# danielzgtg/TTS.cpp

Hardware: AMD Instinct MI355X
Metric: audio-sec/wall-sec (RTF^-1), Parler-TTS-mini v1 Q4_K AR decode + DAC decode (higher is better)
Workload: dtype q4_K weights x q8_K activations (int dot, f32 combine); DAC f16 im2col x f32 weights, f64 accumulate

## Files before the change

### include/tts_hip.h

```cpp
#ifndef TTS_HIP_H
#define TTS_HIP_H

#include <stddef.h>
#include <stdint.h>

#ifdef __cplusplus
extern "C" {
#endif

#define TTS_MAX_DIMS 4
#define TTS_MAX_SRC 4
#define TTS_MAX_OP_PARAMS 16
#define TTS_MAX_NAME 64

enum tts_type {
    TTS_TYPE_F32 = 0,
    TTS_TYPE_F16 = 1,
    TTS_TYPE_Q4_0 = 2,
    TTS_TYPE_Q4_1 = 3,
    TTS_TYPE_Q5_0 = 6,
    TTS_TYPE_Q5_1 = 7,
    TTS_TYPE_Q8_0 = 8,
    TTS_TYPE_Q8_1 = 9,
    TTS_TYPE_Q4_K = 12,
// ... 122 lines not shown
const char * tts_hip_backend_name(tts_hip_backend_t backend);

void * tts_hip_buffer_alloc(tts_hip_backend_t backend, size_t size);
void tts_hip_buffer_free(tts_hip_backend_t backend, void * ptr);
size_t tts_hip_buffer_alignment(void);

int tts_hip_tensor_set(tts_hip_backend_t backend, void * dst_dev, const void * src_host, size_t size);
int tts_hip_tensor_get(tts_hip_backend_t backend, void * dst_host, const void * src_dev, size_t size);
int tts_hip_tensor_copy(tts_hip_backend_t backend, void * dst_dev, const void * src_dev, size_t size);
int tts_hip_copy_stream(tts_hip_backend_t backend, void * dst_dev, const void * src_dev, size_t size);
int tts_hip_plan_stats(tts_tensor * const * nodes, int n_nodes, int mask, int32_t * counts);
int tts_hip_tensor_set_async(tts_hip_backend_t backend, void * dst_dev, const void * src_host, size_t size);
int tts_hip_memset(tts_hip_backend_t backend, void * dst_dev, int value, size_t size);
int tts_hip_synchronize(tts_hip_backend_t backend);

int tts_hip_weight_set(tts_hip_backend_t backend, tts_tensor * t, const void * src_host);
int tts_hip_weight_get(tts_hip_backend_t backend, const tts_tensor * t, void * dst_host);
int tts_hip_quantize(tts_hip_backend_t backend, int type, const float * x_dev, void * dst_dev, int64_t rows, int64_t K);
void tts_repack_q4_K(const void * src, void * dst, int64_t nblocks, int inverse);
void tts_repack_q4_K_tiled(const void * src, void * dst, int64_t nrows, int64_t nb, int inverse);

int tts_hip_supports_op(const tts_tensor * node);
int tts_hip_graph_compute(tts_hip_backend_t backend, tts_tensor * const * nodes, int n_nodes);
int tts_hip_graph_prepare(tts_hip_backend_t backend, tts_tensor * const * nodes, int n_nodes, int slot);
int tts_hip_graph_launch(tts_hip_backend_t backend, int slot);

enum tts_hip_option {
    TTS_HIP_OPT_FUSION = 0,
    TTS_HIP_OPT_PROFILE_GEMV = 1,
    TTS_HIP_OPT_GRAPHS = 2,
    TTS_HIP_OPT_CONV_F32ACC = 3,
    TTS_HIP_OPT_CONVT_LDS = 4,
    TTS_HIP_OPT_ATTN_SPLIT = 5,
    TTS_HIP_OPT_KV_PREFETCH = 6,
    TTS_HIP_OPT_KV_PREFETCH_BLOCKS = 7,
    TTS_HIP_OPT_Q4K_TILE_BYTES = 8,
    TTS_HIP_OPT_GEMV_DEBUG = 10,
    TTS_HIP_OPT_CONV_SPLIT = 12,
    TTS_HIP_OPT_GEMV_UNIQUE = 11,
    TTS_HIP_OPT_GEMV_KS = 13,
    TTS_HIP_OPT_ATTN_FUSED = 14,
    TTS_HIP_OPT_GEMM_Q8 = 18,
    TTS_HIP_OPT_BGEMM_F32 = 19,
    TTS_HIP_OPT_CU_PARTITION = 20,
    TTS_HIP_OPT_Q4K_DUAL_BYTES = 16,
    TTS_HIP_OPT_GEMV_RSPLIT = 17,
    TTS_HIP_OPT_ATTN_PV16 = 15,
    TTS_HIP_OPT_GEMV_PREQUANT = 21,
    TTS_HIP_OPT_GEMV_KRELAY = 22,
    TTS_HIP_OPT_ATTN_KS = 23,
    TTS_HIP_OPT_ATTN_PV8 = 24,
    TTS_HIP_OPT_GEMV_KRELAY_LOOP = 26,
    TTS_HIP_OPT_GEMV_Q80_PRO = 27,
    TTS_HIP_OPT_GEMV_Q80_SLAB = 28,
    TTS_HIP_OPT_GEMV_Q80_RW = 29,
    TTS_HIP_OPT_GEMM_Q8_STAGED = 30,
    TTS_HIP_OPT_GEMV_KR_INKERNEL = 31,
    TTS_HIP_OPT_GEMV_F32_WIDE = 32,
    TTS_HIP_OPT_ATTN_PV_MP = 33,
    TTS_HIP_OPT_GEMM_KR_INKERNEL = 35,
    TTS_HIP_OPT_GEMM_KR_CT2 = 36,
    TTS_HIP_OPT_GEMM_KR_NW = 34,
    TTS_HIP_OPT_GEMV_NW_MIN = 25,
    TTS_HIP_OPT_GEMM_KR_XCD = 38,
    TTS_HIP_OPT_GEMM_KR_CP = 39,
    TTS_HIP_OPT_GEMM_KR_WALK = 40,
    TTS_HIP_OPT_GEMM_PF = 41,
    TTS_HIP_OPT_GEMM_PF_NW = 42,
    TTS_HIP_OPT_ATTN_ONE = 43,
    TTS_HIP_OPT_GEMV_KR_TAIL = 44,
    TTS_HIP_OPT_GEMV_Q50_SLAB = 45,
    TTS_HIP_OPT_GEMV_Q50_RW = 46,
    TTS_HIP_OPT_GEMM_Q5 = 47,
    TTS_HIP_OPT_GEMM_Q5_STAGED = 48,
    TTS_HIP_OPT_GEMV_Q40_SLAB = 49,
    TTS_HIP_OPT_GEMV_Q40_RW = 50,
    TTS_HIP_OPT_GEMM_Q4_0 = 51,
    TTS_HIP_OPT_GEMM_Q4_0_STAGED = 52,
    TTS_HIP_OPT_CONV_VFMA = 53,
    TTS_HIP_OPT_CONV_TILE96 = 54,
    TTS_HIP_OPT_CONV_PACK = 55,
    TTS_HIP_OPT_CONVT_PACK = 56,
    TTS_HIP_OPT_CONV_XREG = 57,
    TTS_HIP_OPT_COALESCE = 37,
};
enum tts_fuse_bits {
    TTS_FUSE_LN = 1, TTS_FUSE_GROUP = 2, TTS_FUSE_KV = 4, TTS_FUSE_EPI = 8, TTS_FUSE_HEADS = 16, TTS_FUSE_ATTN = 32,
    TTS_FUSE_LSTM = 64,
    TTS_FUSE_SNAKE = 128,
    TTS_FUSE_EMBED = 256,
    TTS_FUSE_CONV = 512,
    TTS_FUSE_ADAIN = 1024,
    TTS_FUSE_XATTN = 2048,
    TTS_FUSE_MCPY = 4096,
    TTS_FUSE_CONTREAD = 8192
};
int tts_hip_set_option(tts_hip_backend_t backend, int option, int value);
int tts_hip_attn_decode(tts_hip_backend_t backend, const tts_tensor * q, const tts_tensor * k, const tts_tensor * v,
                        const float * mask, int64_t mbs, float scale, float * out, float * out2, const int64_t * koff,
                        const int64_t * voff, const int64_t * moff, const int32_t * pseq);
int tts_hip_coalesce_stats(int device, int64_t * out, int n);
void tts_hip_coalesce_set_wait(int us);
int tts_hip_coalesce_enable(int on);
#define TTS_HIP_HOOK_FAULT_WEIGHT_SET 1
int tts_hip_test_hook(int hook, int value);
int tts_hip_install_crash_handler(void);
int tts_hip_gemv_stats(tts_hip_backend_t backend, int type, double * ms, int64_t * launches, double * bytes, int reset);
int tts_hip_greedy_step(tts_hip_backend_t backend, const float * logits, int32_t B, int32_t NH, int32_t V, int32_t step,
                        int32_t bos, int32_t eos, int32_t * eos_seen, int32_t * hist, int32_t * next);
typedef struct tts_sampling {
    float temperature;
    float top_p;
    float repetition_penalty;
    int32_t top_k;
    int32_t do_sample;
    int32_t pad_;
    uint64_t seed;
} tts_sampling;
void tts_sampling_default(tts_sampling * cfg);
uint32_t tts_sampler_call_seed(uint64_t seed, int32_t stream, int64_t call);
int tts_sampler_sample(const tts_sampling * cfg, const float * logits, int32_t NH, int32_t V, uint32_t call_seed, int32_t * last,
                       int32_t * count, int32_t * out);
int tts_hip_sample_step(tts_hip_backend_t backend, const float * logits, int32_t B, int32_t NH, int32_t V, const tts_sampling * cfg,
                        int64_t call, int32_t * rep_state, int32_t step, int32_t bos, int32_t eos, int32_t * eos_seen, int32_t * hist,
                        int32_t * next);
int tts_sampling_device_ok(const tts_sampling * cfg, int32_t V);
int tts_hip_counters(tts_hip_backend_t backend, int64_t * out, int n);

int tts_hip_gemv(tts_hip_backend_t backend, int type, const void * w, const float * x, float * y,
                 int64_t K, int64_t N, int64_t M);
int tts_hip_gemv_ex(tts_hip_backend_t backend, int type, const void * w, const float * x, float * y,
                    int64_t K, int64_t N, int64_t M, int32_t wflags);
int tts_hip_gemv_res(tts_hip_backend_t backend, int type, const void * w, const float * x, float * y, const float * res,
                     int64_t K, int64_t N, int64_t M, int32_t wflags);

typedef struct tts_backend_iface {
    void * ctx;
    const char * name;
    void * (*alloc)(void * ctx, size_t size);
    void (*free)(void * ctx, void * ptr);
    int (*set)(void * ctx, void * dst, const void * src, size_t size);
    int (*set_tensor)(void * ctx, tts_tensor * t, const void * src);
    int (*get)(void * ctx, void * dst, const void * src, size_t size);
    int (*memset)(void * ctx, void * dst, int value, size_t size);
    int (*compute)(void * ctx, tts_tensor * const * nodes, int n_nodes);
    int (*synchronize)(void * ctx);
    int (*prepare)(void * ctx, tts_tensor * const * nodes, int n_nodes, int slot);
    int (*launch)(void * ctx, int slot);
    int (*set_async)(void * ctx, void * dst, const void * src, size_t size);
    int (*copy)(void * ctx, void * dst, const void * src, size_t size);
    int (*greedy_step)(void * ctx, const float * logits, int B, int NH, int V, int step, int bos, int eos, int32_t * eos_seen,
                       int32_t * hist, int32_t * next);
    int (*sample_step)(void * ctx, const float * logits, int B, int NH, int V, const tts_sampling * cfg, int64_t call, int32_t * rep_state,
                       int step, int bos, int eos, int32_t * eos_seen, int32_t * hist, int32_t * next);
} tts_backend_iface;

int tts_hip_backend_iface(tts_hip_backend_t backend, tts_backend_iface * out);

#ifdef __cplusplus
}
#endif

#endif
```

### tts.cpp_amd/csrc/backend.hip

```cpp
#include <cmath>
#include <atomic>
#include <cstring>
#include <map>
#include <mutex>
#include <thread>

#include "hip_internal.h"
#include <hip/hip_ext.h>

#include <dlfcn.h>
#include <execinfo.h>
#include <fcntl.h>
#include <signal.h>
#include <unistd.h>

using namespace tts;


static void build_gelu_table(uint16_t * t) {
    const float GELU_COEF_A = 0.044715f;
    const float SQRT_2_OVER_PI = 0.79788456080286535587989211986876f;
    for (int i = 0; i < 65536; ++i) {
        const float x = fp16_to_fp32_host((uint16_t)i);
        const float g = 0.5f * x * (1.0f + tanhf(SQRT_2_OVER_PI * x * (1.0f + GELU_COEF_A * x * x)));
// ... 79 lines not shown
}
void conv_pack_freed(const tts_hip_backend * be, const void * p, size_t n) {
    if (g_packs_n.load(std::memory_order_acquire) == 0) return;
    const char * a = (const char *)p;
    std::vector<float *> dead;
    {
        std::lock_guard<std::mutex> lk(g_reg_mu);
        for (auto it = g_packs.begin(); it != g_packs.end();) {
            const char * w = (const char *)it->first.w;
            if (be ? it->first.be == be : (w >= a && w < a + n)) {
                dead.push_back(it->second.img);
                g_packs_bytes.fetch_sub(it->first.floats() * sizeof(float), std::memory_order_relaxed);
                it = g_packs.erase(it);
            } else {
                ++it;
            }
        }
        if (g_packs.empty()) g_packs_lo.store(UINTPTR_MAX), g_packs_hi.store(0);
        g_packs_n.store(g_packs.size(), std::memory_order_release);
    }
    if (dead.empty()) return;
    hipDeviceSynchronize();
    for (float * c : dead) hipFree(c);
}
bool buffer_lookup(const void * p, const char ** base, size_t * size) {
    std::lock_guard<std::mutex> lk(g_reg_mu);
    auto it = g_buffers.upper_bound((const char *)p);
    if (it == g_buffers.begin()) return false;
    --it;
    if ((const char *)p >= it->first + it->second.size) return false;
    if (base) *base = it->first;
    if (size) *size = it->second.size;
    return true;
}
}

extern "C" {

int tts_hip_coalesce_enable(int on) { return tts::g_coalesce_on.exchange(on ? 1 : 0); }

int tts_hip_device_count(void) {
    int n = 0;
    if (hipGetDeviceCount(&n) != hipSuccess) return 0;
    return n;
}

tts_hip_backend_t tts_hip_backend_init(int device) {
    int n = tts_hip_device_count();
    if (device < 0 || device >= n) return nullptr;
    if (hipSetDevice(device) != hipSuccess) return nullptr;
    auto * be = new tts_hip_backend();
    be->device = device;
    TTS_HIP_CHECK(hipStreamCreateWithFlags(&be->stream, hipStreamNonBlocking));
    TTS_HIP_CHECK(hipStreamCreateWithFlags(&be->cap_stream, hipStreamNonBlocking));
    TTS_HIP_CHECK(hipStreamCreateWithFlags(&be->pf_stream, hipStreamNonBlocking));
    TTS_HIP_CHECK(hipEventCreateWithFlags(&be->co_ev, hipEventDisableTiming));
    TTS_HIP_CHECK(hipEventCreateWithFlags(&be->pf_fork, hipEventDisableTiming));
    TTS_HIP_CHECK(hipEventCreateWithFlags(&be->pf_join, hipEventDisableTiming));
    hipDeviceProp_t prop;
    TTS_HIP_CHECK(hipGetDeviceProperties(&prop, device));
    snprintf(be->name, sizeof(be->name), "HIP%d(%s)", device, prop.gcnArchName);
    be->cu_total = prop.multiProcessorCount > 0 ? prop.multiProcessorCount : 256;
    be->cus = be->cu_total;
    TTS_HIP_CHECK(hipMalloc((void **)&be->scratch, kScratchBytes));
    be->scratch_size = kScratchBytes;
    TTS_HIP_CHECK(hipMalloc((void **)&be->shadow, kShadowBytes));
    be->shadow_size = kShadowBytes;
    be->hoist_size = (size_t)8 << 20;
    TTS_HIP_CHECK(hipMalloc(&be->hoist, be->hoist_size));
    TTS_HIP_CHECK(hipMalloc((void **)&be->lstm_buf, kLstmFloats * sizeof(float)));
    TTS_HIP_CHECK(hipMalloc((void **)&be->attn_buf, kAttnFloats * sizeof(float)));
    be->attn_floats = kAttnFloats;
    TTS_HIP_CHECK(hipMalloc((void **)&be->vec_scratch, kVecScratchFloats * sizeof(float)));
    be->conv_stage_floats = (size_t)8 << 20;
    TTS_HIP_CHECK(hipMalloc((void **)&be->conv_stage, be->conv_stage_floats * sizeof(float)));
    if (const char * e = getenv("TTS_HIP_OPT_CONV_VFMA"))
        if (e[0] >= '0' && e[0] <= '2' && !e[1]) be->conv_vfma = e[0] - '0';
    if (const char * e = getenv("TTS_HIP_OPT_CONV_PACK"))
        if (e[0] >= '0' && e[0] <= '1' && !e[1]) be->conv_pack = e[0] - '0';
    if (const char * e = getenv("TTS_HIP_OPT_CONVT_PACK"))
        if (e[0] >= '0' && e[0] <= '1' && !e[1]) be->convt_pack = e[0] - '0';
    if (const char * e = getenv("TTS_HIP_OPT_CONV_XREG"))
        if (e[0] >= '0' && e[0] <= '1' && !e[1]) be->conv_xreg = e[0] - '0';
    be->conv_part_doubles = (size_t)8 << 20;
    TTS_HIP_CHECK(hipMalloc((void **)&be->conv_part, be->conv_part_doubles * sizeof(double)));
    be->lstm_floats = kLstmFloats;
    TTS_HIP_CHECK(hipMalloc((void **)&be->argmax_keys, kArgmaxRows * sizeof(unsigned long long)));
    TTS_HIP_CHECK(hipMalloc((void **)&be->argmax_counts, kArgmaxRows * sizeof(unsigned)));
    TTS_HIP_CHECK(hipMemset(be->argmax_keys, 0, kArgmaxRows * sizeof(unsigned long long)));
    TTS_HIP_CHECK(hipMemset(be->argmax_counts, 0, kArgmaxRows * sizeof(unsigned)));
    TTS_HIP_CHECK(hipHostMalloc((void **)&be->pin, kPinBytes, hipHostMallocDefault));
    be->pin_size = kPinBytes;
    for (auto & e : be->plan_ev) TTS_HIP_CHECK(hipEventCreateWithFlags(&e, hipEventDisableTiming));
    std::vector<uint16_t> tab(65536);
    build_gelu_table(tab.data());
    TTS_HIP_CHECK(hipMalloc((void **)&be->gelu_table, 65536 * sizeof(uint16_t)));
    TTS_HIP_CHECK(hipMemcpy(be->gelu_table, tab.data(), 65536 * sizeof(uint16_t), hipMemcpyHostToDevice));
    return be;
}

void tts_hip_backend_free(tts_hip_backend_t be) {
    if (!be) return;
    tts::coalesce_backend_gone(be);
    hipSetDevice(be->device);
    hipStreamSynchronize(be->stream);
    tts::conv_pack_freed(be, nullptr, 0);
    for (auto & p : be->ev_pending) {
        hipEventDestroy(p.first);
        hipEventDestroy(p.second);
    }
    for (auto e : be->ev_free) hipEventDestroy(e);
    for (auto & r : be->pin_pending) hipEventDestroy(r.ev);
    for (auto e : be->pin_events) hipEventDestroy(e);
    for (auto e : be->plan_ev) hipEventDestroy(e);
    hipHostFree(be->pin);
    if (be->rb_host) hipHostFree(be->rb_host);
    hipFree(be->scratch);
    hipFree(be->shadow);
    hipFree(be->argmax_keys);
    hipFree(be->argmax_counts);
    hipFree(be->lstm_buf);
    hipFree(be->hoist);
    hipFree(be->attn_buf);
    hipFree(be->vec_scratch);
    hipFree(be->conv_stage);
    hipFree(be->conv_part);
    hipFree(be->gelu_table);
    if (be->sample_cand) hipFree(be->sample_cand);
    if (be->repack_tmp) hipFree(be->repack_tmp);
    for (char * r : be->repack_retired) hipFree(r);
    if (be->attn_stage) hipFree(be->attn_stage);
    for (auto & ex : be->gsig_exec)
        if (ex) hipGraphExecDestroy(ex);
    for (auto & ex : be->pexec)
        if (ex) hipGraphExecDestroy(ex);
    hipStreamDestroy(be->stream);
    hipStreamDestroy(be->cap_stream);
    hipStreamDestroy(be->pf_stream);
    hipEventDestroy(be->pf_fork);
    hipEventDestroy(be->pf_join);
    hipEventDestroy(be->co_ev);
    delete be;
}

const char * tts_hip_backend_name(tts_hip_backend_t be) { return be ? be->name : "HIP(null)"; }

int tts_hip_device_memory(int device, size_t * free_bytes, size_t * total_bytes) {
    if (device < 0 || device >= tts_hip_device_count()) return TTS_STATUS_NO_DEVICE;
    int prev = 0;
    hipGetDevice(&prev);
    hipSetDevice(device);
    size_t f = 0, t = 0;
    const hipError_t e = hipMemGetInfo(&f, &t);
    hipSetDevice(prev);
    if (e != hipSuccess) return TTS_STATUS_FAILED;
    if (free_bytes) *free_bytes = f;
    if (total_bytes) *total_bytes = t;
    return 0;
}

void * tts_hip_event_new(int device) {
    if (device < 0 || device >= tts_hip_device_count()) return nullptr;
    hipSetDevice(device);
    hipEvent_t ev = nullptr;
    if (hipEventCreateWithFlags(&ev, hipEventDisableTiming) != hipSuccess) return nullptr;
    return (void *)ev;
// ... 618 lines not shown
        case TTS_HIP_OPT_GEMM_Q8_STAGED:
            if (value < 0 || value > 2) return TTS_STATUS_BAD_ARG;
            be->gemm_q8_staged = value;
            return 0;
        case TTS_HIP_OPT_GEMV_Q80_RW:
            if (value < 0 || value > 32 || (value & (value - 1))) return TTS_STATUS_BAD_ARG;
            be->gemv_q80_rw = value;
            return 0;
        case TTS_HIP_OPT_GEMV_Q50_SLAB: be->gemv_q50_slab = value != 0; return 0;
        case TTS_HIP_OPT_GEMV_Q50_RW:
            if (value < 0 || value > 32 || (value & (value - 1))) return TTS_STATUS_BAD_ARG;
            be->gemv_q50_rw = value;
            return 0;
        case TTS_HIP_OPT_GEMM_Q5: be->gemm_q5 = value != 0; return 0;
        case TTS_HIP_OPT_GEMM_Q5_STAGED:
            if (value < 0 || value > 2) return TTS_STATUS_BAD_ARG;
            be->gemm_q5_staged = value;
            return 0;
        case TTS_HIP_OPT_GEMV_Q40_SLAB: be->gemv_q40_slab = value != 0; return 0;
        case TTS_HIP_OPT_GEMV_Q40_RW:
            if (value < 0 || value > 32 || (value & (value - 1))) return TTS_STATUS_BAD_ARG;
            be->gemv_q40_rw = value;
            return 0;
        case TTS_HIP_OPT_GEMM_Q4_0: be->gemm_q4_0 = value != 0; return 0;
        case TTS_HIP_OPT_GEMM_Q4_0_STAGED:
            if (value < 0 || value > 2) return TTS_STATUS_BAD_ARG;
            be->gemm_q4_0_staged = value;
            return 0;
        case TTS_HIP_OPT_ATTN_KS: be->attn_ks = value; return 0;
        case TTS_HIP_OPT_GEMV_NW_MIN: be->gemv_nw_min = value; return 0;
        case TTS_HIP_OPT_ATTN_PV8: be->attn_pv8 = value != 0; return 0;
        case TTS_HIP_OPT_GEMM_KR_CT2: be->gemm_kr_ct2 = value != 0; return 0;
        case TTS_HIP_OPT_GEMM_KR_INKERNEL: be->gemm_kr_ink = value < 0 ? 0 : value; return 0;
        case TTS_HIP_OPT_ATTN_PV_MP: be->attn_pv_mp = value == 2 ? 2 : value != 0; return 0;
        case TTS_HIP_OPT_ATTN_ONE:
            if (value < 0 || value > 2) return TTS_STATUS_BAD_ARG;
            be->attn_one = value;
            return 0;
        case TTS_HIP_OPT_GEMV_KR_TAIL:
            if (value < 0 || value > 4) return TTS_STATUS_BAD_ARG;
            be->gemv_kr_tail = value;
            return 0;
        case TTS_HIP_OPT_GEMM_KR_NW: be->gemm_kr_nw = value == 8 ? 8 : 4; return 0;
        case TTS_HIP_OPT_GEMM_Q8: be->gemm_q8 = value != 0; return 0;
        case TTS_HIP_OPT_CU_PARTITION: {
            const int count = value & 0xFF, index = (value >> 8) & 0xFF;
            const bool inter = (value >> 16) & 1;
            hipSetDevice(be->device);
            TTS_HIP_CHECK(hipStreamSynchronize(be->stream));
            hipStream_t ns = nullptr;
            if (count <= 1) {
                TTS_HIP_CHECK(hipStreamCreateWithFlags(&ns, hipStreamNonBlocking));
                be->cus = be->cu_total;
            } else {
                if (index >= count) return TTS_STATUS_BAD_ARG;
                std::vector<uint32_t> mask((be->cu_total + 31) / 32, 0u);
                const int per = be->cu_total / count;
                int n = 0;
                for (int c = 0; c < be->cu_total; ++c) {
                    const bool on = inter ? (c % count == index) : (c / per == index && c < per * count);
                    if (on) mask[c / 32] |= 1u << (c % 32), ++n;
                }
                if (hipExtStreamCreateWithCUMask(&ns, (uint32_t)mask.size(), mask.data()) != hipSuccess) return TTS_STATUS_FAILED;
                be->cus = n;
            }
            TTS_HIP_CHECK(hipStreamDestroy(be->stream));
            be->stream = ns;
            for (auto & ex : be->gsig_exec)
                if (ex) hipGraphExecDestroy(ex), ex = nullptr;
            for (auto & g : be->gsig) g = 0;
            return 0;
        }
        case TTS_HIP_OPT_BGEMM_F32: be->bgemm_f32 = value != 0; return 0;
        case TTS_HIP_OPT_GEMV_F32_WIDE: be->gemv_f32_wide = value != 0; return 0;
        case TTS_HIP_OPT_GEMV_DEBUG: be->gemv_dbg = value; return 0;
        case TTS_HIP_OPT_GEMV_UNIQUE: be->gemv_unique = value != 0; return 0;
        case TTS_HIP_OPT_GEMV_KS: be->gemv_ks_tiles = value > 0 ? value : 0; return 0;
        case TTS_HIP_OPT_COALESCE: be->co_member = value != 0; return 0;
        case TTS_HIP_OPT_GEMM_KR_XCD: be->gemm_kr_xcd = value != 0; return 0;
        case TTS_HIP_OPT_GEMM_KR_CP: be->gemm_kr_cp = value != 0; return 0;
        case TTS_HIP_OPT_GEMM_KR_WALK: be->gemm_kr_walk = value < 0 ? 0 : value; return 0;
        case TTS_HIP_OPT_GEMM_PF: be->gemm_pf = value < 0 ? 0 : value; return 0;
        case TTS_HIP_OPT_GEMM_PF_NW: be->gemm_pf_nw = value == 8 ? 8 : 4; return 0;
        case TTS_HIP_OPT_KV_PREFETCH_BLOCKS: be->kv_prefetch_blocks = value > 0 ? value : 1; return 0;
        default: return TTS_STATUS_BAD_ARG;
    }
}

extern "C" int tts_hip_counters(tts_hip_backend_t be, int64_t * out, int n) {
    if (!be || !out) return TTS_STATUS_BAD_ARG;
    const int64_t v[10] = {be->graph_updates, be->graph_instantiations, be->lstm_chains, be->lstm_steps, be->plan_wait_ns,
                           be->cap_plan_ns, be->cap_launch_ns, be->cap_update_ns, (int64_t)g_packs_n.load(), (int64_t)g_packs_bytes.load()};
    int k = 0;
    for (; k < n && k < 10; ++k) out[k] = v[k];
    return k;
}

extern "C" int tts_hip_gemv_stats(tts_hip_backend_t be, int type, double * ms, int64_t * launches, double * bytes, int reset) {
    if (!be) return TTS_STATUS_BAD_ARG;
    hipSetDevice(be->device);
    TTS_HIP_CHECK(hipStreamSynchronize(be->stream));
    for (size_t i = 0; i < be->ev_pending.size(); ++i) {
        float t = 0;
        TTS_HIP_CHECK(hipEventElapsedTime(&t, be->ev_pending[i].first, be->ev_pending[i].second));
        const int ty = be->ev_type[i];
        be->gemv_ms[ty] += t;
        be->gemv_launches[ty] += 1;
        be->gemv_bytes[ty] += be->ev_bytes[i];
        be->ev_free.push_back(be->ev_pending[i].first);
        be->ev_free.push_back(be->ev_pending[i].second);
    }
    be->ev_pending.clear();
    be->ev_bytes.clear();
    be->ev_type.clear();
    double a = 0, c = 0;
    int64_t b = 0;
    for (int ty = 0; ty < TTS_TYPE_COUNT; ++ty) {
        if (type >= 0 && ty != type) continue;
        a += be->gemv_ms[ty];
        b += be->gemv_launches[ty];
        c += be->gemv_bytes[ty];
    }
    if (ms) *ms = a;
    if (launches) *launches = b;
    if (bytes) *bytes = c;
    if (reset) {
        for (int ty = 0; ty < TTS_TYPE_COUNT; ++ty) {
            be->gemv_ms[ty] = 0;
            be->gemv_launches[ty] = 0;
            be->gemv_bytes[ty] = 0;
        }
    }
    return 0;
}

static void * hb_alloc(void * c, size_t n) { return tts_hip_buffer_alloc((tts_hip_backend_t)c, n); }
static void hb_free(void * c, void * p) { tts_hip_buffer_free((tts_hip_backend_t)c, p); }
static int hb_set(void * c, void * d, const void * s, size_t n) { return tts_hip_tensor_set((tts_hip_backend_t)c, d, s, n); }
static int hb_set_tensor(void * c, tts_tensor * t, const void * s) { return tts_hip_weight_set((tts_hip_backend_t)c, t, s); }
static int hb_get(void * c, void * d, const void * s, size_t n) { return tts_hip_tensor_get((tts_hip_backend_t)c, d, s, n); }
static int hb_memset(void * c, void * d, int v, size_t n) { return tts_hip_memset((tts_hip_backend_t)c, d, v, n); }
static int hb_compute(void * c, tts_tensor * const * nodes, int n) { return tts_hip_graph_compute((tts_hip_backend_t)c, nodes, n); }
static int hb_sync(void * c) { return tts_hip_synchronize((tts_hip_backend_t)c); }
static int hb_prepare(void * c, tts_tensor * const * nodes, int n, int slot) {
    return tts_hip_graph_prepare((tts_hip_backend_t)c, nodes, n, slot);
}
static int hb_launch(void * c, int slot) { return tts_hip_graph_launch((tts_hip_backend_t)c, slot); }
static int hb_set_async(void * c, void * d, const void * s, size_t n) { return tts_hip_tensor_set_async((tts_hip_backend_t)c, d, s, n); }
static int hb_copy(void * c, void * d, const void * s, size_t n) { return tts_hip_tensor_copy((tts_hip_backend_t)c, d, s, n); }
static int hb_greedy(void * c, const float * l, int B, int NH, int V, int step, int bos, int eos, int32_t * seen, int32_t * hist, int32_t * next) {
    return tts_hip_greedy_step((tts_hip_backend_t)c, l, B, NH, V, step, bos, eos, seen, hist, next);
}
static int hb_sample(void * c, const float * l, int B, int NH, int V, const tts_sampling * cfg, int64_t call, int32_t * rep, int step, int bos,
                     int eos, int32_t * seen, int32_t * hist, int32_t * next) {
    return tts_hip_sample_step((tts_hip_backend_t)c, l, B, NH, V, cfg, call, rep, step, bos, eos, seen, hist, next);
}

extern "C" int tts_hip_backend_iface(tts_hip_backend_t be, tts_backend_iface * out) {
    if (!be || !out) return TTS_STATUS_BAD_ARG;
    out->ctx = be;
    out->name = be->name;
    out->alloc = hb_alloc;
    out->free = hb_free;
    out->set = hb_set;
    out->set_tensor = hb_set_tensor;
    out->get = hb_get;
    out->memset = hb_memset;
    out->compute = hb_compute;
    out->synchronize = hb_sync;
    out->prepare = hb_prepare;
    out->launch = hb_launch;
    out->set_async = hb_set_async;
    out->copy = hb_copy;
    out->greedy_step = hb_greedy;
    out->sample_step = hb_sample;
    return 0;
}
// ... 1 lines not shown
```

### tts.cpp_amd/csrc/graph_exec.hip

```cpp
#include <algorithm>
#include <cstring>
#include <deque>
#include <unordered_map>
#include <vector>

#include <array>

#include "hip_internal.h"
#include <chrono>

using namespace tts;

namespace tts {
void launch_kv_prefetch(tts_hip_backend * be, hipStream_t st, const TD & t, int pdim, int blocks);
void launch_gemv_q4K_xattn(tts_hip_backend * be, const GemvJob & j, const XAttnArgs & a);
void launch_attn_decode(tts_hip_backend * be, const TD & q, const TD & k, const TD & v, const float * mask, float scale,
                        float * out, int hd, int P, int H, int n, int B, float * out2, int64_t obs = -1, int64_t mbs = 0,
                        const int64_t * koff = nullptr, const int64_t * voff = nullptr, const int64_t * moff = nullptr,
                        const int * pseq = nullptr);
void launch_attn_bias(tts_hip_backend * be, const TD & q, const TD & k, const TD & v, const float * bias, const float * mask,
                      float scale, float * out, int P, int H, int n);
void launch_layernorm(tts_hip_backend * be, const tts_tensor * dst, const tts_tensor * x, const float * w, const float * b,
                      float eps, bool rms);
}
// ... 28 lines not shown
    return t->nb[0] == es && t->nb[1] == t->nb[0] * (size_t)(t->ne[0] / tts_blck_size(t->type)) &&
           t->nb[2] == t->nb[1] * (size_t)t->ne[1] && t->nb[3] == t->nb[2] * (size_t)t->ne[2];
}

bool persistent_mem(const tts_tensor * t) {
    for (int hop = 0; t && hop < 8; ++hop) {
        if (t->op == TTS_OP_NONE || (t->flags & TTS_FLAG_PERSIST)) return true;
        if (!is_view(t->op)) return false;
        t = t->view_src ? t->view_src : t->src[0];
    }
    return false;
}

bool is_1d_f32(const tts_tensor * t, int64_t n) {
    return t->type == TTS_TYPE_F32 && t->ne[0] == n && t->ne[1] == 1 && t->ne[2] == 1 && t->ne[3] == 1 && t->nb[0] == 4;
}

float opf(const tts_tensor * t, int i) {
    float f;
    memcpy(&f, &t->op_params[i], 4);
    return f;
}

static int64_t nel(const tts_tensor * t) { return t->ne[0] * t->ne[1] * t->ne[2] * t->ne[3]; }

bool is_gemv(const tts_tensor * n) {
    const tts_tensor * a = n->src[0];
    const tts_tensor * b = n->src[1];
    if (a->ne[2] != 1 || a->ne[3] != 1) return false;
    if (b->type != TTS_TYPE_F32 || b->nb[0] != 4) return false;
    if (b->ne[2] * b->ne[3] != 1 && !(b->nb[2] == b->nb[1] * (size_t)b->ne[1] && b->nb[3] == b->nb[2] * (size_t)b->ne[2]))
        return false;
    if (n->nb[0] != 4 || (n->ne[2] * n->ne[3] != 1 && !(n->nb[2] == n->nb[1] * (size_t)n->ne[1] && n->nb[3] == n->nb[2] * (size_t)n->ne[2])))
        return false;
    if (a->nb[0] != tts_type_size(a->type)) return false;
    if ((a->type == TTS_TYPE_F16 || a->type == TTS_TYPE_F32) && b->ne[1] * b->ne[2] * b->ne[3] > 64) return false;
    if (a->type == TTS_TYPE_F16 && b->ne[1] * b->ne[2] * b->ne[3] > 8 && a->ne[0] % 8 == 0 && (b->nb[1] % 16) == 0 &&
        ((uintptr_t)b->data % 16) == 0 && (a->nb[1] % 16) == 0)
        return false;
    switch (a->type) {
        case TTS_TYPE_Q4_K:
        case TTS_TYPE_Q6_K: return a->ne[0] % 256 == 0;
        case TTS_TYPE_Q8_0:
        case TTS_TYPE_Q5_0:
        case TTS_TYPE_Q4_0: return a->ne[0] % 32 == 0;
        case TTS_TYPE_F32:
        case TTS_TYPE_F16: return a->ne[0] % 4 == 0 && (b->nb[1] % 16) == 0 && ((uintptr_t)b->data % 16) == 0;
        default: return false;
    }
}

struct GemvTarget {
    float * y;
    int64_t ycs, yrs;
    int32_t rg = 0, nrep = 1;
    int64_t rgs = 0, rep = 0;
    const tts_tensor * yt = nullptr;
};

struct Item {
    enum Kind { GEMV, ATTN, LN, LSTM, SNAKE, EMBED, CONV, ADAIN, MCPY, RINT, NODE, COPY } kind;
    const void * cp_src = nullptr;
    void * cp_dst = nullptr;
    size_t cp_bytes = 0;
    tts_tensor node{};
    const tts_tensor * rope = nullptr;
    std::vector<const tts_tensor *> mms;
    std::vector<GemvTarget> tgt;
    int epi = EPI_NONE;
    const tts_tensor * res = nullptr;
    bool ln = false;
    const tts_tensor *lnx = nullptr, *lnw = nullptr, *lnb = nullptr, *lndst = nullptr;
    float lneps = 0.f;
    bool lnrms = false;
    bool x_shadow = false;
    const tts_tensor * snake_one = nullptr;
    const tts_tensor * snake_mask = nullptr;
    bool gather_t = false;
    const tts_tensor * gt_codes = nullptr;
    const tts_tensor * xsrc = nullptr;
    bool shadow = false;
    int xattn = -1;
    bool fused = false;
    const tts_tensor *q = nullptr, *k = nullptr, *v = nullptr, *mask = nullptr, *out = nullptr;
    const tts_tensor * bias = nullptr;
    bool stage = false;
    float scale = 1.f;
    const tts_tensor *x = nullptr, *w = nullptr, *b = nullptr, *dst = nullptr;
    float eps = 0.f;
    bool rms = false;
    std::vector<const tts_tensor *> terms;
    int lkind = 0;
    LstmStepArgs ls{}, ls2{};
    bool lpair = false;
    const tts_tensor *lfinal = nullptr, *lfinal2 = nullptr;
    const float *lhist = nullptr, *lhist2 = nullptr;
    int64_t lHd = 0, lT = 0;
    const void * lstash_src[4] = {};
    void * lstash_dst[4] = {};
    size_t lstash_bytes = 0;
    Conv1dArgs conv{};
    AdainArgs adain{};
    bool rint_cpy = false;
    int rint = 1;
};

struct SmallIdx {
    int inl[3];
    std::vector<int> more;
    int n = 0;
    void push_back(int v) {
        if (n < 3) inl[n] = v;
        else more.push_back(v);
        ++n;
    }
    size_t size() const { return (size_t)n; }
    int operator[](size_t i) const { return i < 3 ? inl[i] : more[i - 3]; }
    struct iter {
        const SmallIdx * s;
        size_t i;
        int operator*() const { return (*s)[i]; }
        iter & operator++() {
            ++i;
            return *this;
        }
        bool operator!=(const iter & o) const { return i != o.i; }
        bool operator==(const iter & o) const { return i == o.i; }
        using iterator_category = std::input_iterator_tag;
        using value_type = int;
        using difference_type = std::ptrdiff_t;
        using pointer = const int *;
        using reference = int;
    };
    iter begin() const { return {this, 0}; }
    iter end() const { return {this, (size_t)n}; }
};

template <typename V>
struct PtrMap {
    struct Entry {
        const tts_tensor * first;
        V second;
    };
    std::vector<Entry> entries;
    std::vector<int32_t> slots;
    size_t mask_ = 0;
    void reserve(size_t n) {
        size_t cap = 64;
        while (cap < 2 * n) cap <<= 1;
        slots.assign(cap, -1);
        mask_ = cap - 1;
        entries.clear();
        entries.reserve(n);
    }
    size_t slot(const tts_tensor * k) const {
        uint64_t h = (uint64_t)(uintptr_t)k * 0x9E3779B97F4A7C15ull;
        size_t i = (size_t)(h >> 32) & mask_;
        while (slots[i] >= 0 && entries[slots[i]].first != k) i = (i + 1) & mask_;
        return i;
    }
    V & operator[](const tts_tensor * k) {
        if (slots.empty()) reserve(64);
        size_t i = slot(k);
        if (slots[i] < 0) {
            if (2 * (entries.size() + 1) > slots.size()) {
                std::vector<Entry> old;
// ... 52 lines not shown
            if (is_view(nodes[k]->op) || std::find(own.begin(), own.end(), k) != own.end()) continue;
            if (overlap(nodes[k], t)) return true;
        }
        return false;
    }
    const tts_tensor * sole_consumer(const tts_tensor * t) {
        auto it = consumers.find(t);
        if (it == consumers.end() || it->second.size() != 1 || uses[t] != 1) return nullptr;
        if (nodes[it->second[0]] == t) return nullptr;
        return nodes[it->second[0]];
    }
    int next_real(int i) {
        for (int j = i + 1; j < n; ++j)
            if (!is_view(nodes[j]->op)) return j;
        return -1;
    }

    void build(tts_tensor * const * nodes_, int n_) {
        const auto t_build0 = std::chrono::steady_clock::now();
        nodes = nodes_;
        n = n_;
        act.assign(n, 0);
        index.reserve((size_t)n);
        consumers.reserve((size_t)n * 2);
        for (int i = 0; i < n; ++i) {
            index[nodes[i]] = i;
            for (int s = 0; s < TTS_MAX_SRC; ++s) {
                const tts_tensor * x = nodes[i]->src[s];
                if (!x) continue;
                bool dup = false;
                for (int s2 = 0; s2 < s; ++s2) dup |= nodes[i]->src[s2] == x;
                if (dup) continue;
                consumers[x].push_back(i);
            }
        }
        for (int i = 0; i < n; ++i)
            if (read_after(nodes[i]) && !is_view(nodes[i]->op)) consumers[nodes[i]].push_back(i);
        static const bool timing = getenv("TTS_PLAN_TIMING") != nullptr;
        auto t_last = t_build0;
        char tbuf[512];
        int tlen = 0;
        auto tmark = [&](const char * what) {
            if (!timing) return;
            const auto now = std::chrono::steady_clock::now();
            tlen += snprintf(tbuf + tlen, sizeof(tbuf) - (size_t)tlen, " %s %.3f", what, std::chrono::duration<double, std::milli>(now - t_last).count());
            t_last = now;
        };
        tmark("index");
        if (mask & TTS_FUSE_LSTM) try_lstm();
        tmark("lstm");
        if (mask & TTS_FUSE_MCPY)
            for (int i = n - 1; i >= 0; --i)
                if (act[i] == 0 && nodes[i]->op == TTS_OP_CONCAT) try_rint(i);
        tmark("rint");
        if (mask & TTS_FUSE_EMBED)
            for (int i = n - 1; i >= 0; --i)
                if (act[i] == 0 && nodes[i]->op == TTS_OP_ADD) try_embed(i);
        tmark("embed");
        for (int i = 0; i < n; ++i) {
            if (act[i] != 0) continue;
            const tts_tensor * t = nodes[i];
            switch (t->op) {
                case TTS_OP_NORM:
                    if ((mask & TTS_FUSE_ADAIN) && try_adain(i)) break;
                    if (mask & TTS_FUSE_LN) try_ln(i);
                    break;
                case TTS_OP_RMS_NORM: if (mask & TTS_FUSE_LN) try_ln(i); break;
                case TTS_OP_SOFT_MAX: if (mask & TTS_FUSE_ATTN) try_attn(i); break;
                case TTS_OP_ADD: if (mask & TTS_FUSE_SNAKE) try_snake(i); break;
                case TTS_OP_IM2COL: if (mask & TTS_FUSE_CONV) try_conv(i); break;
                case TTS_OP_CPY: if (mask & TTS_FUSE_MCPY) try_mcpy(i); break;
                case TTS_OP_CONT: if (mask & TTS_FUSE_EMBED) try_gather_t(i); break;
                case TTS_OP_MUL_MAT:
                    if (!((mask & TTS_FUSE_HEADS) && try_heads(i)) && (mask & (TTS_FUSE_GROUP | TTS_FUSE_KV | TTS_FUSE_EPI))) try_gemv(i);
                    break;
                default: break;
            }
        }
        tmark("patterns");
        if (mask & TTS_FUSE_CONTREAD) skip_cont_reads();
        if (mask & TTS_FUSE_LN) fuse_ln_into_gemv();
        link_attn_shadow();
        if (mask & TTS_FUSE_XATTN) fuse_xattn();
        tmark("post");
        if (timing) fprintf(stderr, "plan %d nodes ms:%s\n", n, tbuf);
    }

    void link_attn_shadow() {
        for (int i = 0; i < n; ++i) {
            const int a = act[i];
            if (a <= 0 || items[a - 1].kind != Item::ATTN) continue;
            const int nx = next_real(i);
            if (nx < 0 || act[nx] <= 0) continue;
            Item & A = items[a - 1];
            Item & G = items[act[nx] - 1];
            if (A.bias) continue;
            if (G.kind != Item::GEMV || G.ln || G.mms[0]->src[0]->type != TTS_TYPE_Q4_K) continue;
            const tts_tensor * x = G.mms[0]->src[1];
            if (x->data != A.out->data || !contiguous(x) || tbytes(x) != tbytes(A.out)) continue;
            A.shadow = G.x_shadow = true;
        }
    }

    void fuse_xattn() {
        for (size_t ai = 0; ai < items.size(); ++ai) {
            Item & A = items[ai];
            if (A.kind != Item::ATTN || A.bias || A.k->ne[1] > 64 || A.q->ne[0] != 64 || A.q->ne[1] != 1) continue;
            const tts_tensor * Q = A.q;
            const tts_tensor * t = Q;
            int hops = 0;
            while (t && is_view(t->op) && t->src[0] && hops < 4) {
                if (uses[t->src[0]] != 1) break;
                t = t->src[0];
                ++hops;
            }
            if (!t || t->op != TTS_OP_MUL_MAT || uses[t] != 1) continue;
            const int gi = act[index[t]];
            if (gi <= 0) continue;
            Item & G = items[gi - 1];
            if (G.kind != Item::GEMV || G.mms.size() != 1 || G.mms[0] != t || G.epi != EPI_NONE || G.res || G.xattn >= 0) continue;
            const tts_tensor * W = t->src[0];
            const int64_t H = Q->ne[2], B = Q->ne[3];
            if (W->type != TTS_TYPE_Q4_K || (W->flags & TTS_FLAG_TILED) || W->ne[0] > 1024 || W->ne[1] != 64 * H ||
                t->ne[1] * t->ne[2] * t->ne[3] != B) continue;
            if (G.tgt[0].y != (float *)t->data || G.tgt[0].ycs != W->ne[1] || G.tgt[0].yrs != 1) continue;
            if (Q->data != t->data || Q->nb[0] != 4 || Q->nb[2] != 256 || (int64_t)Q->nb[3] != 4 * W->ne[1]) continue;
            if (A.k->ne[2] != H || A.v->ne[2] != H || B % A.k->ne[3] || B % A.v->ne[3]) continue;
            if (A.mask && A.mask->ne[0] != A.k->ne[1]) continue;
            const int g_node = index[t], o_node = index[A.out];
            bool clear = g_node < o_node;
            for (int i = g_node + 1; clear && i < o_node; ++i)
                if (act[i] > 0 || (act[i] == 0 && !is_view(nodes[i]->op))) clear = false;
            if (!clear) continue;
            G.xattn = (int)ai;
            A.fused = true;
        }
    }

    void skip_cont_reads() {
        for (int i = 0; i < n; ++i) {
            const tts_tensor * C = nodes[i];
            if (act[i] != 0 || C->op != TTS_OP_CONT || !C->src[0]) continue;
            const tts_tensor * s = C->src[0];
            if (s->type != C->type || !contiguous(s) || !contiguous(C) || uses[C] != 1) continue;
            if (s->ne[0] != C->ne[0] || s->ne[1] != C->ne[1] || s->ne[2] != C->ne[2] || s->ne[3] != C->ne[3]) continue;
            if (C->flags & (TTS_FLAG_OUTPUT | TTS_FLAG_PERSIST)) continue;
            const int r = next_real(i);
            if (r < 0 || act[r] != 0) continue;
            const tts_tensor * R = nodes[r];
            if (R->src[0] != C || (R->op != TTS_OP_ROPE && R->op != TTS_OP_UNARY)) continue;
            bool other = false;
            for (int si = 1; si < TTS_MAX_SRC; ++si) other |= R->src[si] == C;
            bool same = R->data == s->data && R->type == s->type;
            for (int d = 0; d < 4 && same; ++d) same = R->ne[d] == s->ne[d] && R->nb[d] == s->nb[d];
            if (other || (overlap(R, s) && !same)) continue;
            Item it;
            it.kind = Item::NODE;
            it.node = *R;
            it.node.src[0] = const_cast<tts_tensor *>(s);
            act[i] = -1;
            act[r] = add_item(std::move(it));
        }
    }

    void fuse_ln_into_gemv() {
        for (int i = 0; i < n; ++i) {
            const int a = act[i];
            if (a <= 0 || items[a - 1].kind != Item::LN) continue;
            const int nx = next_real(i);
            if (nx < 0 || act[nx] <= 0) continue;
            Item & L = items[a - 1];
            Item & G = items[act[nx] - 1];
            if (G.kind != Item::GEMV || G.ln || G.mms[0]->src[1] != L.dst) continue;
            const int wt = G.mms[0]->src[0]->type;
            const tts_tensor * B = G.mms[0]->src[1];
            if (!wtype_q8k_act(wt) && !(wtype_q80_act(wt) && q80pro && B->ne[1] * B->ne[2] * B->ne[3] <= 8)) continue;
            const int64_t K = L.dst->ne[0];
            if (K % 256 || K > 4096) continue;
            if (((uintptr_t)L.w->data & 15) || (L.b && ((uintptr_t)L.b->data & 15)) || (L.dst->nb[1] & 15)) continue;
            G.ln = true;
            G.lnx = L.x;
            G.lnw = L.w;
            G.lnb = L.b;
// ... 1480 lines not shown
    }
    const tts_tensor * member(const BatchCtx & bc, const tts_tensor * t, int k) {
        if (k == 0 || !t) return t;
        auto * e = pos.find(t);
        if (!e) return nullptr;
        const int64_t c = e->second;
        const tts_tensor * nd = bc.mnodes[k][c >> 5];
        const int slot = (int)(c & 31);
        const tts_tensor * r = slot == 31 ? nd : slot == 30 ? nd->view_src : nd->src[slot];
        return r && r->op == t->op && r->type == t->type ? r : nullptr;
    }
};
static const tts_tensor * co_member(const BatchCtx & bc, const tts_tensor * t, int k) {
    return ((CoMap *)bc.comap)->member(bc, t, k);
}
static const tts_tensor * mem_root(const tts_tensor * t) { return t && t->view_src ? t->view_src : t; }
static bool owned_mem(const tts_tensor * t) {
    const tts_tensor * r = mem_root(t);
    return r && (r->op == TTS_OP_NONE || (r->flags & TTS_FLAG_PERSIST) || persistent_mem(r));
}
static bool input_mem(const tts_tensor * t) {
    const tts_tensor * r = mem_root(t);
    return r && r->op == TTS_OP_NONE && (r->flags & TTS_FLAG_INPUT) != 0;
}

static void batch_td(const BatchCtx & bc, TD & t) {
    const int64_t s = bc.stride(t.data);
    t.data = bc.win(t.data);
    if (s) {
        t.ne[3] = bc.N;
        t.nb[3] = s;
    }
}
static int batch_n(const tts_hip_backend * be) { return be->bat ? be->bat->N : 1; }

static int run_attn_item(tts_hip_backend * be, const Item & it, const ItemTab * tab = nullptr) {
    TD q = make_td(it.q), k = make_td(it.k), v = make_td(it.v);
    float * out = (float *)it.out->data;
    const float * mask = it.mask ? (const float *)it.mask->data : nullptr;
    int B = (int)it.q->ne[3], P = (int)it.k->ne[1];
    if (it.bias) {
        if (be->bat) return TTS_STATUS_UNSUPPORTED;
        const size_t ob = tbytes(it.out);
        if (it.stage && be->attn_stage_size < ob) {
            if (be->stream == be->cap_stream) return TTS_STATUS_ALLOC_FAILED;
            if (be->attn_stage) be->repack_retired.push_back((char *)be->attn_stage);
            be->attn_stage = nullptr;
            be->attn_stage_size = 0;
            const size_t nbytes = (ob + (1u << 20) - 1) & ~(size_t)((1u << 20) - 1);
            if (hipMalloc((void **)&be->attn_stage, nbytes) != hipSuccess) {
                (void)hipGetLastError();
                return TTS_STATUS_ALLOC_FAILED;
            }
            be->attn_stage_size = nbytes;
        }
        launch_attn_bias(be, q, k, v, (const float *)it.bias->data, mask, it.scale, it.stage ? be->attn_stage : out, P, (int)it.q->ne[2],
                         (int)it.q->ne[1]);
        if (it.stage) TTS_HIP_CHECK(hipMemcpyAsync(out, be->attn_stage, ob, hipMemcpyDeviceToDevice, be->stream));
        return 0;
    }
    int64_t obs = -1, mbs = it.mask && it.mask->ne[3] > 1 ? (int64_t)(it.mask->nb[3] / 4) : 0;
    if (const BatchCtx * bc = be->bat) {
        batch_td(*bc, q);
        if (tab && tab->koff) k.ne[3] = bc->N, k.nb[3] = 0;
        else batch_td(*bc, k);
        if (tab && tab->voff) v.ne[3] = bc->N, v.nb[3] = 0;
        else batch_td(*bc, v);
        obs = bc->stride(out) / 4;
        out = bc->win(out);
        if (mask && !(tab && tab->moff)) {
            mbs = bc->stride(mask) / 4;
            mask = bc->win(mask);
        }
        B = bc->N;
        if (tab && tab->pseq) P = tab->pmax;
    }
    float * out2 = it.shadow && tbytes(it.out) * (size_t)batch_n(be) <= be->shadow_size ? be->shadow : nullptr;
    launch_attn_decode(be, q, k, v, mask, it.scale, out, (int)it.q->ne[0], P, (int)it.q->ne[2], (int)it.q->ne[1], B, out2, obs, mbs,
                       tab ? tab->koff : nullptr, tab ? tab->voff : nullptr, tab ? tab->moff : nullptr, tab ? tab->pseq : nullptr);
    return 0;
}

static int run_gemv_item(tts_hip_backend * be, const Item & it, const Item * xattn = nullptr, const ItemTab * tab = nullptr,
                         const ItemTab * xtab = nullptr) {
    const tts_tensor * mm0 = it.mms[0];
    const tts_tensor * a0 = mm0->src[0];
    tts_tensor bx;
    if (it.xsrc) {
        bx = *mm0->src[1];
        bx.data = it.xsrc->data;
    }
    const tts_tensor * b = it.xsrc ? &bx : mm0->src[1];
    GemvJob j;
    j.wtype = a0->type;
    j.K = a0->ne[0];
    j.N = a0->ne[1];
    j.M = nel(b) / b->ne[0];
    j.w_row_bytes = (int64_t)a0->nb[1];
    j.x = (const float *)b->data;
    j.xcs = (int64_t)(b->nb[1] / 4);
    const BatchCtx * bc = be->bat;
    const int64_t NB = bc ? bc->N : 1;
    j.epi = it.epi;
    j.gelu = be->gelu_table;
    if (it.res) {
        j.res = (const float *)it.res->data;
        j.rcs = (int64_t)(it.res->nb[1] / 4);
    }
    const bool q80pro = wtype_q80_act(j.wtype) && j.K % QK_K == 0 && j.M <= 8 && (it.ln || be->gemv_q80_pro);
    if (wtype_q8k_act(j.wtype) || q80pro) {
        j.pro = it.ln ? PRO_LN : PRO_QUANT;
        j.tiled = (a0->flags & TTS_FLAG_TILED) ? 1 : 0;
        if (it.ln) {
            j.x = (const float *)it.lnx->data;
            j.xcs = (int64_t)(it.lnx->nb[1] / 4);
            j.lnw = (const float *)it.lnw->data;
            j.lnb = it.lnb ? (const float *)it.lnb->data : nullptr;
            j.eps = it.lneps;
            j.rms = it.lnrms ? 1 : 0;
            j.lnout = (float *)it.lndst->data;
            j.locs = (int64_t)(it.lndst->nb[1] / 4);
        }
        auto span_y = [&](size_t k, const char *& y0, const char *& y1) {
            const tts_tensor * mm = it.mms[k];
            const int64_t Mm = mm->ne[1] * mm->ne[2] * mm->ne[3];
            y0 = (const char *)it.tgt[k].y;
            y1 = y0 + 4 * (size_t)((Mm - 1) * it.tgt[k].ycs + (mm->ne[0] - 1) * it.tgt[k].yrs + 1);
        };
        const bool xs = it.x_shadow && (size_t)(4 * j.K * j.M * NB) <= be->shadow_size;
        if (xs) {
            j.x = be->shadow;
            j.xcs = j.K;
        }
        const char * x0 = (const char *)j.x;
        const char * x1 = x0 + 4 * (size_t)((j.M - 1) * j.xcs + j.K);
        const char * l0 = (const char *)j.lnout;
        const char * l1 = l0 ? l0 + 4 * (size_t)((j.M - 1) * j.locs + j.K) : nullptr;
        bool x_hit = l0 && l0 < x1 && x0 < l1;
        for (size_t k = 0; k < it.tgt.size(); ++k) {
            const char *y0, *y1;
            span_y(k, y0, y1);
            x_hit |= y0 < x1 && x0 < y1;
            if (l0 && y0 < l1 && l0 < y1) j.lnout = nullptr;
        }
        if (bc) {
            if (!xs) {
                j.xcs = bc->stride(j.x) / 4;
                j.x = bc->win(j.x);
            }
            if (j.lnout) {
                j.locs = bc->stride(j.lnout) / 4;
                j.lnout = bc->win(j.lnout);
            }
            j.M = NB;
        }
        x_hit |= ((uintptr_t)j.x & 15) != 0 || (j.xcs & 3) != 0;
        if (x_hit) {
            if (!ensure_scratch(be, (size_t)(4 * j.K * j.M))) return TTS_STATUS_ALLOC_FAILED;
            launch_copy_cols(be, (float *)be->scratch, j.x, j.K, j.xcs, j.M);
            be->aq.src = nullptr;
            j.x = (const float *)be->scratch;
            j.xcs = j.K;
        }
    } else {
        if (it.ln) return TTS_STATUS_UNSUPPORTED;
        if (bc) {
            j.xcs = bc->stride(j.x) / 4;
            j.x = bc->win(j.x);
            j.M = NB;
        }
        int st = prepare_act(be, j.wtype, j.x, j.xcs, j.K, j.M, j.aq);
        if (st) return st;
    }
    if (bc && j.res) {
        j.rcs = bc->stride(j.res) / 4;
        j.res = bc->win(j.res);
    }
    const bool tmp = a0->type == TTS_TYPE_Q4_K && !(a0->flags & TTS_FLAG_REPACKED);
    if (xattn) {
        const Item & A = *xattn;
        TD k = make_td(A.k), v = make_td(A.v);
        const char * o0 = (const char *)A.out->data;
        const char * o1 = o0 + tbytes(A.out);
        const float * xm = bc ? (const float *)(it.ln ? it.lnx->data : b->data) : j.x;
        const int64_t xmcs = bc ? 0 : j.xcs, mm = bc ? 1 : j.M;
        const char * x0 = (const char *)xm;
        const char * x1 = x0 + 4 * (size_t)((mm - 1) * xmcs + j.K);
        const bool ok = !tmp && !j.tiled && j.wtype == TTS_TYPE_Q4_K && j.K <= 1024 && j.N == 64 * A.q->ne[2] && k.nb[0] == 4 &&
                        (k.nb[1] % 16) == 0 && (k.nb[2] % 16) == 0 && (k.nb[3] % 16) == 0 && ((uintptr_t)k.data % 16) == 0 &&
                        A.k->ne[1] >= 1 && A.k->ne[1] <= 64 && !(o0 < x1 && x0 < o1) && contiguous(A.out);
        if (ok) {
            GemvJob jj = j;
            jj.nmat = 1;
            jj.W[0] = (const uint8_t *)weight_ptr(be, a0);
            jj.Y[0] = nullptr;
            if (jj.lnout) {
                const char * l0 = it.ln ? (const char *)it.lndst->data : (const char *)jj.lnout;
                const char * l1 = l0 + 4 * (size_t)((mm - 1) * (bc ? 0 : j.locs) + j.K);
                if (l0 < o1 && o0 < l1) jj.lnout = nullptr;
            }
            XAttnArgs xa;
            xa.k = k;
            xa.v = v;
            xa.mask = A.mask ? (const float *)A.mask->data : nullptr;
            xa.scale = A.scale;
            xa.out = (float *)A.out->data;
            xa.out2 = A.shadow && tbytes(A.out) * (size_t)NB <= be->shadow_size ? be->shadow : nullptr;
            xa.P = (int)A.k->ne[1];
            xa.H = (int)A.q->ne[2];
            xa.B = (int)A.q->ne[3];
            if (bc) {
                if (xtab && xtab->koff) xa.k.ne[3] = NB, xa.k.nb[3] = 0;
                else batch_td(*bc, xa.k);
                if (xtab && xtab->voff) xa.v.ne[3] = NB, xa.v.nb[3] = 0;
                else batch_td(*bc, xa.v);
                if (xtab && xtab->moff) {
                    xa.moff = xtab->moff;
                } else {
                    xa.mbs = bc->stride(xa.mask) / 4;
                    xa.mask = bc->win(xa.mask);
                }
                xa.koff = xtab ? xtab->koff : nullptr;
                xa.voff = xtab ? xtab->voff : nullptr;
                if (xtab && xtab->pseq) xa.pseq = xtab->pseq, xa.P = xtab->pmax;
                xa.obs = bc->stride(xa.out) / 4;
                xa.out = bc->win(xa.out);
                xa.B = (int)NB;
            }
            launch_gemv_q4K_xattn(be, jj, xa);
            return 0;
        }
    }
    bool all_tl = j.wtype == TTS_TYPE_Q4_K && !tmp, any_tiled = false;
    int64_t rows = 0;
    for (const tts_tensor * mm : it.mms) {
        const int f = mm->src[0]->flags;
        all_tl &= (f & (TTS_FLAG_TILED | TTS_FLAG_TILED_COPY)) != 0;
        any_tiled |= (f & TTS_FLAG_TILED) != 0;
        rows += mm->src[0]->ne[1];
    }
    const bool use_copy = all_tl && (any_tiled || (j.M >= 8 && rows >= 2048 && j.K >= 2048));
    if (use_copy) j.tiled = 1;
    size_t k = 0;
    while (k < it.mms.size()) {
        GemvJob jj = j;
        jj.nmat = 0;
        jj.hetero = 0;
        jj.roff[0] = 0;
        if (bc && tab && tab->yoff) {
            jj.yoff = tab->yoff + k * NB;
            jj.yoff_ld = (int32_t)NB;
            jj.yoff_mats = (int32_t)((uint32_t)tab->yoff_mats >> k);
        }
        while (k < it.mms.size() && jj.nmat < GEMV_MAX_MATS) {
            const tts_tensor * a = it.mms[k]->src[0];
            if (jj.nmat > 0 && a->ne[1] != jj.N && !jj.tiled) break;
            if (it.tgt[k].rg > 0 && jj.rep_mat >= 0) break;
            if (jj.nmat > 0 && a->ne[1] != jj.N) jj.hetero = 1;
            jj.W[jj.nmat] = (const uint8_t *)weight_ptr(be, a, use_copy && !(a->flags & TTS_FLAG_TILED));
            jj.Y[jj.nmat] = bc ? bc->win(it.tgt[k].y) : it.tgt[k].y;
            jj.ycs[jj.nmat] = bc ? bc->stride(it.tgt[k].y) / 4 : it.tgt[k].ycs;
            jj.yrs[jj.nmat] = it.tgt[k].yrs;
            if (it.tgt[k].rg > 0) {
                jj.rep_mat = jj.nmat;
                jj.yrg = it.tgt[k].rg;
                jj.yrgs = it.tgt[k].rgs;
                jj.nrep = it.tgt[k].nrep;
                jj.yrep = it.tgt[k].rep;
            }
            if (jj.nmat == 0) jj.N = a->ne[1];
            jj.roff[jj.nmat + 1] = jj.roff[jj.nmat] + a->ne[1];
            jj.nmat++;
            k++;
            if (tmp) break;
        }
        if (jj.hetero) jj.N = 0;
        if (jj.wtype == TTS_TYPE_Q6_K && !gemv_q6k_ok(jj)) return TTS_STATUS_UNSUPPORTED;
        launch_gemv_job(be, jj);
    }
    if (xattn) return run_attn_item(be, *xattn, xtab);
    return 0;
}

__global__ void k_gather_t(float * __restrict__ dst, const char * __restrict__ w, int64_t wnb1, const char * __restrict__ ids,
                           int64_t inb1, int64_t T, int64_t C) {
    for (int64_t e = (int64_t)blockIdx.x * blockDim.x + threadIdx.x; e < T * C; e += (int64_t)gridDim.x * blockDim.x) {
        const int64_t c = e / T, t = e - c * T;
        const int32_t id = *(const int32_t *)(ids + t * inb1);
        dst[e] = *(const float *)(w + (int64_t)id * wnb1 + 4 * c);
    }
}

static void launch_gather_t(tts_hip_backend * be, const tts_tensor * dst, const tts_tensor * w, const tts_tensor * ids) {
    const int64_t T = dst->ne[0], C = dst->ne[1];
    int64_t g = (T * C + 255) / 256;
    if (g > 4096) g = 4096;
    hipLaunchKernelGGL(k_gather_t, dim3((unsigned)g), dim3(256), 0, be->stream, (float *)dst->data, (const char *)w->data,
                       (int64_t)w->nb[1], (const char *)ids->data, (int64_t)ids->nb[1], T, C);
    TTS_HIP_CHECK(hipGetLastError());
}

static int run_node(tts_hip_backend * be, const tts_tensor * n);

static bool batch_tensor(const BatchCtx & bc, const tts_tensor * t, tts_tensor & o) {
    o = *t;
    const int64_t s = bc.stride(t->data);
    o.data = bc.win(t->data);
    if (!s) return true;
    if (t->ne[3] != 1) return false;
    o.ne[3] = bc.N;
    o.nb[3] = (size_t)s;
    return true;
}

static int run_node_coalesced(tts_hip_backend * be, const tts_tensor * n) {
    const BatchCtx & bc = *be->bat;
    bool per_slice = false;
    switch (n->op) {
        case TTS_OP_ADD: case TTS_OP_SUB: case TTS_OP_MUL: case TTS_OP_DIV: case TTS_OP_SQR: case TTS_OP_SQRT: case TTS_OP_SIN:
        case TTS_OP_COS: case TTS_OP_SCALE: case TTS_OP_CLAMP: case TTS_OP_LEAKY_RELU: case TTS_OP_UNARY: case TTS_OP_ROUND:
        case TTS_OP_MOD: case TTS_OP_NORM: case TTS_OP_RMS_NORM: case TTS_OP_CONT: case TTS_OP_CPY: case TTS_OP_DUP:
            per_slice = true;
            break;
        case TTS_OP_CONCAT: per_slice = n->op_params[0] < 3; break;
        default: break;
    }
    tts_tensor t, srcs[TTS_MAX_SRC];
    if (per_slice && !owned_mem(n) && bc.stride(n->data) && batch_tensor(bc, n, t)) {
        for (int i = 0; i < TTS_MAX_SRC && per_slice; ++i) {
            const tts_tensor * x = n->src[i];
            if (!x) continue;
            if (input_mem(x) || (!owned_mem(x) && !bc.stride(x->data))) {
                per_slice = false;
                break;
            }
            per_slice = batch_tensor(bc, x, srcs[i]);
            if ((n->op == TTS_OP_CONT || n->op == TTS_OP_CPY || n->op == TTS_OP_DUP) && !bc.stride(x->data)) per_slice = false;
            t.src[i] = &srcs[i];
        }
        if (per_slice) return launch_op(be, &t);
    }
    BatchCtx * keep = be->bat;
    be->bat = nullptr;
    int st = 0;
    auto addr = [&](const tts_tensor * x, int k) -> void * {
        if (!owned_mem(x)) return bc.reloc(x->data, k);
        const tts_tensor * m = co_member(bc, x, k);
        return m ? m->data : nullptr;
    };
    for (int k = 0; k < bc.N && st == 0; ++k) {
        t = *n;
        t.data = addr(n, k);
        for (int i = 0; i < TTS_MAX_SRC; ++i) {
            if (!n->src[i]) continue;
            srcs[i] = *n->src[i];
            srcs[i].data = addr(n->src[i], k);
            if (!srcs[i].data) st = TTS_STATUS_FAILED;
            t.src[i] = &srcs[i];
        }
        if (!t.data) st = TTS_STATUS_FAILED;
        if (st == 0) st = run_node(be, &t);
    }
    be->bat = keep;
    return st;
}

static int run_node(tts_hip_backend * be, const tts_tensor * n) {
    if (be->bat) return run_node_coalesced(be, n);
    if (n->op == TTS_OP_MUL_MAT) {
        const tts_tensor * a = n->src[0], * b = n->src[1];
        if (a->ne[0] != b->ne[0] || b->ne[2] % a->ne[2] || b->ne[3] % a->ne[3]) return TTS_STATUS_UNSUPPORTED;
        if (is_gemv(n)) {
            Item it;
            it.kind = Item::GEMV;
            it.mms.push_back(n);
            it.tgt.push_back(GemvTarget{(float *)n->data, (int64_t)(n->nb[1] / 4), 1});
            it.tgt.back().yt = n;
            return run_gemv_item(be, it);
        }
        const int t = n->src[0]->type;
        if (t == TTS_TYPE_F32 || t == TTS_TYPE_F16) return launch_op(be, n);
        return TTS_STATUS_UNSUPPORTED;
    }
    return launch_op(be, n);
}

static int run_item(tts_hip_backend * be, const Item & it, const std::vector<Item> & items) {
    const ItemTab * tab = be->bat ? &be->bat->tabs[&it - items.data()] : nullptr;
    switch (it.kind) {
        case Item::GEMV:
            return run_gemv_item(be, it, it.xattn >= 0 ? &items[it.xattn] : nullptr, tab,
                                 be->bat && it.xattn >= 0 ? &be->bat->tabs[it.xattn] : nullptr);
        case Item::ATTN:
            if (it.fused) return 0;
            return run_attn_item(be, it, tab);
        case Item::LN:
            if (be->bat) {
                tts_tensor d, x;
                if (!batch_tensor(*be->bat, it.dst, d) || !batch_tensor(*be->bat, it.x, x)) return TTS_STATUS_UNSUPPORTED;
                launch_layernorm(be, &d, &x, (const float *)it.w->data, it.b ? (const float *)it.b->data : nullptr, it.eps, it.rms);
                return 0;
            }
            launch_layernorm(be, it.dst, it.x, (const float *)it.w->data, it.b ? (const float *)it.b->data : nullptr, it.eps, it.rms);
            return 0;
        case Item::EMBED:
            if (it.gather_t) launch_gather_t(be, it.dst, it.w, it.gt_codes);
            else launch_embed_sum(be, it.dst, it.terms.data(), (int)it.terms.size(), be->bat, tab);
            return 0;
        case Item::SNAKE:
            launch_snake(be, it.dst, it.x, it.w, it.b, it.snake_one, it.snake_mask);
            return 0;
        case Item::CONV:
            launch_conv1d_fused(be, it.conv);
            return 0;
        case Item::ADAIN:
            launch_adain_snake(be, it.adain);
            return 0;
        case Item::MCPY:
            if (it.rope) launch_rope_multi(be, it.rope, it.x, it.terms.data(), (int)it.terms.size());
            else launch_cpy_multi(be, it.x, it.terms.data(), (int)it.terms.size());
            return 0;
        case Item::RINT:
            launch_repeat_interleave1(be, it.rint_cpy ? &it.node : it.dst, it.x, it.rint);
            return 0;
        case Item::NODE:
            return run_node(be, &it.node);
        case Item::COPY:
            launch_copy_bytes(be, it.cp_dst, it.cp_src, it.cp_bytes);
            return 0;
        case Item::LSTM:
            if (it.lkind & 4)
                for (int g = 0; g < 4; ++g)
                    launch_copy_bytes(be, it.lstash_dst[g], it.lstash_src[g], it.lstash_bytes);
            if (it.lkind & 1) {
                launch_lstm_step(be, it.ls, it.lpair ? &it.ls2 : nullptr);
                be->lstm_steps += it.lpair ? 2 : 1;
            }
            if (it.lkind & 2) {
                launch_lstm_finish(be, it.lfinal, it.lhist, it.lHd, it.lT);
                be->lstm_chains++;
                if (it.lfinal2) {
                    launch_lstm_finish(be, it.lfinal2, it.lhist2, it.lHd, it.lT);
                    be->lstm_chains++;
                }
            }
            return 0;
    }
    return TTS_STATUS_FAILED;
}

bool tts::co_debug() {
    static const bool on = [] {
        const char * e = getenv("TTS_HIP_COALESCE_DEBUG");
        return e && e[0] == '1';
    }();
    return on;
}
#define CO_NO()                                                                                   \
    do {                                                                                          \
        if (tts::co_debug()) fprintf(stderr, "coalesce: step refused at graph_exec.hip:%d\n", __LINE__); \
        return false;                                                                             \
    } while (0)

static bool co_per_slice(const BatchCtx & bc, const tts_tensor * n) {
    switch (n->op) {
        case TTS_OP_ADD: case TTS_OP_SUB: case TTS_OP_MUL: case TTS_OP_DIV: case TTS_OP_SQR: case TTS_OP_SQRT: case TTS_OP_SIN:
        case TTS_OP_COS: case TTS_OP_SCALE: case TTS_OP_CLAMP: case TTS_OP_LEAKY_RELU: case TTS_OP_UNARY: case TTS_OP_ROUND:
        case TTS_OP_MOD: case TTS_OP_NORM: case TTS_OP_RMS_NORM: case TTS_OP_CONT: case TTS_OP_CPY: case TTS_OP_DUP: break;
        case TTS_OP_CONCAT:
            if (n->op_params[0] < 3) break;
            return false;
        default: return false;
    }
    if (owned_mem(n) || !bc.stride(n->data) || n->ne[3] != 1) return false;
    for (int i = 0; i < TTS_MAX_SRC; ++i) {
// ... 661 lines not shown
```

### tts.cpp_amd/csrc/hip_internal.h

```cpp
#pragma once

#include <hip/hip_fp16.h>
#include <hip/hip_runtime.h>

#include <cstdio>
#include <cstdlib>
#include <atomic>
#include <deque>
#include <mutex>
#include <unordered_map>
#include <tuple>
#include <vector>

#include "common.h"

#define TTS_HIP_CHECK(expr)                                                                          \
    do {                                                                                             \
        hipError_t err_ = (expr);                                                                    \
        if (err_ != hipSuccess) {                                                                    \
            fprintf(stderr, "%s:%d: HIP error %s: %s\n", __FILE__, __LINE__, #expr, hipGetErrorString(err_)); \
            abort();                                                                                 \
        }                                                                                            \
    } while (0)

// ... 178 lines not shown
}
#endif

struct ActQuant {
    const void * src = nullptr;
    int64_t K = 0, M = 0;
    int vtype = -1;
    int64_t graph_epoch = -1;
    int8_t * qs = nullptr;
    float * d = nullptr;
    int32_t * bsums = nullptr;
};

enum { EPI_NONE = 0, EPI_GELU = 1, EPI_ADD = 2, EPI_SWIGLU = 3, EPI_SILU_MUL = 4 };
constexpr int GEMV_MAX_MATS = 16;
struct GemvJob {
    int wtype = 0;
    int nmat = 1;
    const uint8_t * W[GEMV_MAX_MATS] = {};
    float * Y[GEMV_MAX_MATS] = {};
    int64_t w_row_bytes = 0, K = 0, N = 0, M = 0;
    int64_t ycs[GEMV_MAX_MATS] = {}, yrs[GEMV_MAX_MATS] = {};
    const float * res = nullptr;
    int64_t rcs = 0;
    int epi = EPI_NONE;
    const uint16_t * gelu = nullptr;
    const float * x = nullptr;
    int64_t xcs = 0;
    ActQuant aq;
    int pro = 0;
    int tiled = 0;
    int hetero = 0;
    int64_t roff[GEMV_MAX_MATS + 1] = {};
    int32_t rep_mat = -1, yrg = 0, nrep = 0;
    int64_t yrgs = 0, yrep = 0;
    int dbg = 0;
    const float * lnw = nullptr;
    const float * lnb = nullptr;
    float eps = 0.f;
    int rms = 0;
    float * lnout = nullptr;
    int64_t locs = 0;
    const char * bq = nullptr;
    int64_t bq_bytes = 0;
    int64_t bq_tile = 0;
    int32_t bq_slot = 0;
    unsigned long long * ts = nullptr;
    const int64_t * yoff = nullptr;
    int32_t yoff_mats = 0, yoff_ld = 0;
    int32_t xcd_cols = 0;
    int32_t kr_tail = 0;
};
enum { KR_TAIL_RES = 1, KR_TAIL_FOLD = 2, KR_TAIL_BESIDE = 4 };
constexpr int KR_FOLD_BYTES = 4 * 4 * (2 * 64 * 16 + 64 * 4);
__host__ __device__ inline int64_t job_roff(const GemvJob & j, int m) { return j.hetero ? j.roff[m] : (int64_t)m * j.N; }
__host__ __device__ inline int64_t job_rows(const GemvJob & j) { return job_roff(j, j.nmat); }
#ifdef TTS_PHASE_TS
#define TTS_TS(job, k)                                                                                            \
    do {                                                                                                          \
        if ((job).ts && (threadIdx.x & 63) == 0)                                                                  \
            (job).ts[((((size_t)blockIdx.z * gridDim.y + blockIdx.y) * gridDim.x + blockIdx.x) * (blockDim.x >> 6) + \
                      (threadIdx.x >> 6)) * 8 +                                                                   \
                     (k)] = __builtin_amdgcn_s_memrealtime();                                                     \
    } while (0)
#else
#define TTS_TS(job, k) \
    do {               \
    } while (0)
#endif
enum { PRO_QUANT = 1, PRO_LN = 2, PRO_COPY = 3 };
struct XAttnArgs {
    TD k, v;
    const float * mask = nullptr;
    float scale = 1.f;
    float * out = nullptr;
    float * out2 = nullptr;
    int P = 0, H = 0, B = 0;
    int64_t obs = 0;
    int64_t mbs = 0;
    const int64_t * koff = nullptr;
    const int64_t * voff = nullptr;
    const int64_t * moff = nullptr;
    const int * pseq = nullptr;
};

constexpr int EMBED_MAX_TERMS = 16;
struct BatchCls {
    const char * b0 = nullptr;
    size_t size = 0;
    char * win = nullptr;
    int64_t stride = 0;
};
struct ItemTab {
    const int64_t * yoff = nullptr;
    int32_t yoff_mats = 0;
    const int64_t *koff = nullptr, *voff = nullptr;
    const int64_t * moff = nullptr;
    const int * pseq = nullptr;
    int pmax = 0;
    const int64_t * ioff[EMBED_MAX_TERMS] = {};
};
struct BatchCtx {
    int N = 0;
    uint64_t key = 0;
    std::vector<BatchCls> cls;
    std::vector<tts_tensor * const *> mnodes;
    std::vector<tts_hip_backend *> mbe;
    int n_nodes = 0;
    bool checked = false;
    int canon = 0;
    bool ragged = false;
    bool differs = false;
    std::vector<ItemTab> tabs;
    void * comap = nullptr;
    const BatchCls * find(const void * p) const {
        const char * c = (const char *)p;
        size_t lo = 0, hi = cls.size();
        while (lo < hi) {
            const size_t m = (lo + hi) / 2;
            if (cls[m].b0 <= c) lo = m + 1;
            else hi = m;
        }
        if (lo == 0) return nullptr;
        const BatchCls & b = cls[lo - 1];
        return c < b.b0 + b.size ? &b : nullptr;
    }
    template <typename T>
    T * win(T * p) const {
        const BatchCls * b = p ? find(p) : nullptr;
        return b ? (T *)(b->win + ((const char *)p - b->b0)) : p;
    }
    int64_t stride(const void * p) const {
        const BatchCls * b = p ? find(p) : nullptr;
        return b ? b->stride : 0;
    }
    template <typename T>
    T * reloc(T * p, int k) const {
        const BatchCls * b = p ? find(p) : nullptr;
        return b ? (T *)(b->win + k * b->stride + ((const char *)p - b->b0)) : p;
    }
};

}

struct tts_hip_backend {
    int device = 0;
    hipStream_t stream = nullptr;
    char name[64] = {0};
    char * scratch = nullptr;
    size_t scratch_size = 0;
    float * shadow = nullptr;
    size_t shadow_size = 0;
    void * hoist = nullptr;
    size_t hoist_size = 0;
    float * attn_buf = nullptr;
    size_t attn_floats = 0;
    int attn_split_minp = 128;
    int attn_ks = 2;
    int attn_pv_mp = 1;
    int attn_one = 1;
    int attn_pv8 = 0;
    int attn_pv_uv16 = 0;
    int attn_fused_minp = 0;
    unsigned long long * argmax_keys = nullptr;
    unsigned * argmax_counts = nullptr;
    int64_t q4k_tile_bytes = 4 << 20;
    int gemv_dbg = 0;
    int gemv_unique = 1;
    int gemm_q8 = 1;
    int64_t cus = 256;
    int cu_total = 256;
    int bgemm_f32 = 1;
    int gemv_f32_wide = 1;
    int gemm_kr_nw = 4;
    int64_t gemv_ks_tiles = 256;
    int gemv_mf_prequant = 1;
    int gemv_kr = 1;
    int gemv_kr_loop = 1;
    int gemv_kr_tail = 1;
    int gemv_q80_pro = 1;
    int gemv_q80_slab = 1;
    int gemv_q80_rw = 0;
    int gemm_q8_staged = 2;
    int gemv_q50_slab = 1;
    int gemv_q50_rw = 0;
    int gemm_q5 = 1;
    int gemm_q5_staged = 2;
    int gemv_q40_slab = 1;
    int gemv_q40_rw = 0;
    int gemm_q4_0 = 1;
    int gemm_q4_0_staged = 2;
    int64_t gemv_kr_ink = 0;
    int gemm_kr_walk = 0;
    int gemm_pf = 64;
    int gemm_pf_nw = 4;
    int gemm_kr_cp = 0;
    int gemm_kr_xcd = 0;
    int gemm_kr_ct2 = 0;
    int64_t gemm_kr_ink = 0;
    int gemv_nw_min = 0;
    int gemv_mf_rsplit = 1;
    int64_t q4k_dual_bytes = 1 << 20;
    void * sample_cand = nullptr;
    size_t sample_cand_size = 0;
    int kv_prefetch_minp = 0;
    int kv_prefetch_blocks = 128;
    hipStream_t pf_stream = nullptr;
    hipEvent_t pf_fork = nullptr, pf_join = nullptr;
    uint8_t * pin = nullptr;
    size_t pin_size = 0, pin_head = 0;
    struct PinRec {
        size_t off, size;
        hipEvent_t ev;
    };
    std::deque<PinRec> pin_pending;
    std::vector<hipEvent_t> pin_events;
    std::mutex pin_mu;
    hipEvent_t plan_ev[2] = {nullptr, nullptr};
    bool plan_ev_pending[2] = {false, false};
    float * lstm_buf = nullptr;
    float * conv_stage = nullptr;
    size_t conv_stage_floats = 0;
    float * vec_scratch = nullptr;
    size_t lstm_floats = 0;
    tts::ActQuant aq;
    int64_t graph_epoch = 0;
    uint16_t * gelu_table = nullptr;
    bool convt_lds = true;
    double * conv_part = nullptr;
    size_t conv_part_doubles = 0;
    int conv_vfma = 1;
    int conv_tile96 = 1;
    int conv_pack = 1;
    int convt_pack = 1;
    int conv_xreg = 1;
    bool capturing = false;
    int conv_split = 1;
    int fusion = 0x3FFF;
    bool profile_gemv = false;
    double gemv_ms[TTS_TYPE_COUNT] = {0};
    int64_t gemv_launches[TTS_TYPE_COUNT] = {0};
    double gemv_bytes[TTS_TYPE_COUNT] = {0};
    std::vector<std::pair<hipEvent_t, hipEvent_t>> ev_pending;
    std::vector<double> ev_bytes;
    std::vector<int> ev_type;
    std::vector<hipEvent_t> ev_free;
    char * repack_tmp = nullptr;
    size_t repack_tmp_size = 0;
    std::vector<char *> repack_retired;
    float * attn_stage = nullptr;
    size_t attn_stage_size = 0;
    bool use_graphs = false;
    static constexpr int N_GSIG = 4;
    uint64_t gsig[N_GSIG] = {};
    hipGraphExec_t gsig_exec[N_GSIG] = {};
    int gsig_next = 0;
    bool conv_f32acc = false;
    int conv_acc_mode = 0;
    hipStream_t cap_stream = nullptr;
    int64_t graph_updates = 0, graph_instantiations = 0;
    int64_t lstm_chains = 0, lstm_steps = 0;
    int64_t plan_wait_ns = 0;
    int64_t cap_plan_ns = 0, cap_launch_ns = 0, cap_update_ns = 0;
    hipGraphExec_t pexec[2] = {nullptr, nullptr};
    tts_tensor * const * plan_nodes[2] = {nullptr, nullptr};
    int plan_n[2] = {0, 0};
    bool plan_eager[2] = {true, true};
    bool plan_prepared[2] = {false, false};
    tts::BatchCtx * bat = nullptr;
    hipEvent_t co_ev = nullptr;
    int64_t * co_tab = nullptr;
    size_t co_tab_bytes = 0;
    int64_t co_prep_ns = 0;
    bool co_member = true;
    struct RbEnt {
        const char * dev;
        size_t bytes, off;
// ... 159 lines not shown
```

### tts.cpp_amd/csrc/k_gemv.hip

```cpp
#include "hip_internal.h"
#include <hip/hip_ext.h>

#include <atomic>
#include <type_traits>

#ifndef TTS_GEMV_EARLY16
#define TTS_GEMV_EARLY16 1
#endif

namespace tts {

__device__ __forceinline__ int dev_nearest_int(float f) {
    const float val = __fadd_rn(f, 12582912.f);
    const int i = __float_as_int(val);
    return (i & 0x007fffff) - 0x00400000;
}

__global__ __launch_bounds__(256) void k_quantize_q8_K(const float * __restrict__ x, int64_t xcs, int64_t K,
                                                       int8_t * __restrict__ qs, float * __restrict__ dout,
                                                       int32_t * __restrict__ s32) {
    const int blk = blockIdx.x;
    const int m = blockIdx.y;
    const int t = threadIdx.x;
    const int64_t nb = K / QK_K;
// ... 1588 lines not shown
    const int P = a.pseq ? a.pseq[b] : a.P;
    const int p = min(lane, P - 1);
    float4 kr[F];
    float vv[VB];
    float mk = 0.f;
    const int bk = b / (a.B / (int)a.k.ne[3]), bv = b / (a.B / (int)a.v.ne[3]);
    const char * kbase = a.k.data + (int64_t)h * a.k.nb[2] + (int64_t)bk * a.k.nb[3] + (a.koff ? a.koff[b] : 0);
    const char * vbase = a.v.data + (int64_t)h * a.v.nb[2] + (int64_t)bv * a.v.nb[3] + (a.voff ? a.voff[b] : 0);
    u32x4 hdr[4], q[4];
    if (wave < NW) {
        const int64_t row = (int64_t)h * HD + wave * 8 + s;
        const uint8_t * wr = j.W[0] + row * j.w_row_bytes;
        auto mid = [&]() {
#pragma unroll
            for (int u = 0; u < 4; ++u) {
                const int64_t bo = (int64_t)min(u, nb - 1) * 144;
                hdr[u] = TTS_WLOAD((const u32x4 *)(wr + bo));
                q[u] = TTS_WLOAD((const u32x4 *)(wr + bo + 16 + l * 16));
            }
        };
        ProOv ov;
        ov.nwaves = NW;
        ov.xcol = j.x + (int64_t)b * j.xcs;
        ov.lncol = j.lnout && h == 0 ? j.lnout + (int64_t)b * j.locs : nullptr;
        q4k_prologue<PRO, 4>(j, nb, xq_s, xd_s, xs_s, nullptr, nullptr, mid, ov);
    } else {
#pragma unroll
        for (int c = 0; c < F; ++c) kr[c] = *(const float4 *)(kbase + (int64_t)p * a.k.nb[1] + 16 * c);
#pragma unroll
        for (int u = 0; u < VB; ++u) vv[u] = *(const float *)(vbase + (int64_t)lane * a.v.nb[1] + (int64_t)min(u, P - 1) * a.v.nb[0]);
        mk = *(a.mask ? a.mask + (a.moff ? a.moff[b] : (int64_t)b * a.mbs) + p : (const float *)kbase);
    }
    __syncthreads();
    if (wave < NW) {
        float sums = 0.f, sumf = 0.f;
#pragma unroll
        for (int u = 0; u < 4; ++u) q4k_block(hdr[u], q[u], xq_s, xs_s, xd_s, min(u, nb - 1), l, u < nb, sums, sumf);
        const float tot = q4k_octet_total(sumf, sums);
        if (l == 0) s_q[wave * 8 + s] = tot;
    }
    __syncthreads();
    if (wave != NW) return;
    double acc = 0.0;
#pragma unroll
    for (int c = 0; c < F; ++c) {
        acc += (double)__fmul_rn(kr[c].x, s_q[4 * c + 0]);
        acc += (double)__fmul_rn(kr[c].y, s_q[4 * c + 1]);
        acc += (double)__fmul_rn(kr[c].z, s_q[4 * c + 2]);
        acc += (double)__fmul_rn(kr[c].w, s_q[4 * c + 3]);
    }
    float w = __fmul_rn((float)acc, a.scale);
    if (a.mask) w = __fadd_rn(w, __fmul_rn(1.0f, mk));
    if (lane >= P) w = -INFINITY;
    float mx = w;
    mx = fmaxf(mx, dpp_f32<DPP_XOR1>(mx));
    mx = fmaxf(mx, dpp_f32<DPP_XOR2>(mx));
    mx = fmaxf(mx, dpp_f32<DPP_HALF_MIRROR>(mx));
    mx = fmaxf(mx, dpp_f32<DPP_MIRROR>(mx));
    mx = fmaxf(fmaxf(__int_as_float(__builtin_amdgcn_readlane(__float_as_int(mx), 0)), __int_as_float(__builtin_amdgcn_readlane(__float_as_int(mx), 16))),
               fmaxf(__int_as_float(__builtin_amdgcn_readlane(__float_as_int(mx), 32)), __int_as_float(__builtin_amdgcn_readlane(__float_as_int(mx), 48))));
    const float e = lane < P ? cr_expf(__fsub_rn(w, mx)) : 0.f;
    double sum = 0.0;
    for (int i = 0; i < P; ++i) sum += (double)__int_as_float(__builtin_amdgcn_readlane(__float_as_int(e), i));
    const float pr = __fmul_rn(e, (float)(1.0 / sum));
    double o = 0.0;
    for (int i0 = 0; i0 < P; i0 += VB) {
        if (i0 > 0) {
#pragma unroll
            for (int u = 0; u < VB; ++u) vv[u] = *(const float *)(vbase + (int64_t)lane * a.v.nb[1] + (int64_t)min(i0 + u, P - 1) * a.v.nb[0]);
            TTS_PIN_LOADS();
        }
#pragma unroll
        for (int u = 0; u < VB; ++u) {
            if (i0 + u >= P) break;
            const float pi = __int_as_float(__builtin_amdgcn_readlane(__float_as_int(pr), i0 + u));
            o += (double)__fmul_rn(pi, vv[u]);
        }
    }
    const int64_t orow = (int64_t)h * HD + lane;
    a.out[(int64_t)b * (a.obs ? a.obs : (int64_t)a.H * HD) + orow] = (float)o;
    if (a.out2) a.out2[(int64_t)b * a.H * HD + orow] = (float)o;
}

void launch_gemv_q4K_xattn(tts_hip_backend * be, const GemvJob & j, const XAttnArgs & a) {
    const dim3 grid((unsigned)a.H, (unsigned)a.B);
    if (j.pro == PRO_LN) hipLaunchKernelGGL(k_gemv_q4K_xattn<PRO_LN>, grid, dim3(576), 0, be->stream, j, a);
    else hipLaunchKernelGGL(k_gemv_q4K_xattn<PRO_QUANT>, grid, dim3(576), 0, be->stream, j, a);
    TTS_HIP_CHECK(hipGetLastError());
}

template <int MC, int PRO = 0>
__global__ __launch_bounds__(256) void k_gemv_q8_0(GemvJob j, int RW) {
    extern __shared__ __attribute__((aligned(16))) char smem[];
    const int nb = (int)(j.K / QK8_0);
    const int mat = blockIdx.y;
    const uint8_t * __restrict__ W = j.W[mat];
    float * Y = j.Y[mat];
    const int64_t row0 = (int64_t)blockIdx.x * RW;
    const int rows = (int)((j.N - row0) < RW ? (j.N - row0) : RW);
    const int M = j.M;
    int8_t * xq_s = (int8_t *)smem;
    float * xd_s = (float *)(smem + al16((size_t)MC * j.K + (PRO ? QK_K : 0)));
    int * s_s = (int *)((char *)xd_s + al16(sizeof(float) * (MC * nb + (PRO ? QK_K / QK8_0 : 0))));
    float * f_s = (float *)((char *)s_s + al16(sizeof(int) * (size_t)RW * nb * MC));
    const int npairs = rows * nb;
    int wv0[8];
    uint16_t dw0;
    {
        const int p = min((int)threadIdx.x, npairs - 1);
        const int r = p / nb, b = p % nb;
        const uint16_t * bp = (const uint16_t *)(W + (row0 + r) * j.w_row_bytes + (int64_t)b * 34);
        dw0 = *gptr(bp);
#pragma unroll
        for (int k = 0; k < 8; ++k) wv0[k] = (int)*gptr(bp + 1 + 2 * k) | ((int)*gptr(bp + 2 + 2 * k) << 16);
    }
    TTS_PIN_LOADS();
    if constexpr (PRO != 0) {
        q4k_prologue<PRO, 16, false, NoMid, true>(j, (int)(j.K / QK_K), xq_s, xd_s, nullptr);
    } else {
        const int4 * src = (const int4 *)j.aq.qs;
        int4 * dst = (int4 *)xq_s;
        const int n16 = (int)((int64_t)M * j.K / 16);
        for (int i = threadIdx.x; i < n16; i += 256) dst[i] = src[i];
        for (int i = threadIdx.x; i < M * nb; i += 256) xd_s[i] = j.aq.d[i];
    }
    __syncthreads();
    for (int p = threadIdx.x; p < npairs; p += 256) {
        const int r = p / nb, b = p % nb;
        float dw;
        int wv[8];
        if (p == (int)threadIdx.x) {
            dw = dev_fp16_to_fp32(dw0);
#pragma unroll
            for (int k = 0; k < 8; ++k) wv[k] = wv0[k];
        } else {
            const uint16_t * bp = (const uint16_t *)(W + (row0 + r) * j.w_row_bytes + (int64_t)b * 34);
            dw = dev_fp16_to_fp32(bp[0]);
#pragma unroll
            for (int k = 0; k < 8; ++k) wv[k] = (int)bp[1 + 2 * k] | ((int)bp[2 + 2 * k] << 16);
        }
#pragma unroll
        for (int m = 0; m < MC; ++m) {
            if (m >= M) break;
            const int4 * xb = (const int4 *)(xq_s + (m * nb + b) * QK8_0);
            const int4 x0 = xb[0], x1 = xb[1];
            int s = __builtin_amdgcn_sdot4(wv[0], x0.x, 0, false);
            s = __builtin_amdgcn_sdot4(wv[1], x0.y, s, false);
            s = __builtin_amdgcn_sdot4(wv[2], x0.z, s, false);
            s = __builtin_amdgcn_sdot4(wv[3], x0.w, s, false);
            s = __builtin_amdgcn_sdot4(wv[4], x1.x, s, false);
            s = __builtin_amdgcn_sdot4(wv[5], x1.y, s, false);
            s = __builtin_amdgcn_sdot4(wv[6], x1.z, s, false);
            s = __builtin_amdgcn_sdot4(wv[7], x1.w, s, false);
            const int o = (r * MC + m) * nb + b;
            s_s[o] = s;
            f_s[o] = __fmul_rn(dw, xd_s[m * nb + b]);
        }
    }
    __syncthreads();
    for (int t = threadIdx.x; t < rows * MC; t += 256) {
        const int r = t / MC, m = t % MC;
        if (m >= M) continue;
        float a = 0.f;
        const int o = (r * MC + m) * nb;
        for (int b = 0; b < nb; ++b) a = __fadd_rn(a, __fmul_rn((float)s_s[o + b], f_s[o + b]));
        gemv_store<MC>(j, mat, row0 + r, m, a);
    }
// ... 806 lines not shown
        j.x = job.x + m0 * job.xcs;
        for (int i = 0; i < job.nmat; ++i) j.Y[i] = job.Y[i] + m0 * job.ycs[i];
        if (job.yoff) j.yoff = job.yoff + m0;
        if (job.res) j.res = job.res + m0 * job.rcs;
        if (j.pro == PRO_LN && j.K > 4 * 1024) {
            fprintf(stderr, "tts_hip: LN-fused Q4_K GEMV with K = %lld > 4096\n", (long long)j.K);
            abort();
        }
        const int64_t nb = j.K / QK_K;
        const int64_t bq = (((j.M * nb + 1) * (2 * QK_K + 32 + 4)) + 1023) & ~(int64_t)1023;
        if (j.K <= be->gemv_kr_ink && !j.dbg) {
            GemvJob ji = j;
            ji.bq = nullptr;
            ji.bq_bytes = bq;
            if (launch_q4k_kr(be, ji)) continue;
        }
        if (be->gemv_mf_prequant && !j.dbg && (size_t)(bq + 4 * j.K * j.M) <= be->scratch_size) {
            j.bq = be->scratch + be->scratch_size - bq;
            j.bq_bytes = bq;
            const dim3 qg((unsigned)((nb + 3) / 4), (unsigned)j.M);
            if (j.pro == PRO_LN) hipLaunchKernelGGL(k_quant_mf<PRO_LN>, qg, dim3(64), 0, be->stream, j);
            else hipLaunchKernelGGL(k_quant_mf<PRO_QUANT>, qg, dim3(64), 0, be->stream, j);
            TTS_HIP_CHECK(hipGetLastError());
            j.pro = PRO_COPY;
            j.lnout = nullptr;
            if (!launch_q4k_kr(be, j)) launch_q4k_mf_pro<PRO_COPY, 16>(be, j);
            continue;
        }
        if (j.pro == PRO_LN) launch_q4k_mf_pro<PRO_LN, 16>(be, j);
        else launch_q4k_mf_pro<PRO_QUANT, 16>(be, j);
    }
}

static size_t q4k_kr_lds(int64_t bq_bytes, bool sw) { return (size_t)((bq_bytes + 15) & ~15) + (sw ? 2 * 64 * 36 * 4 + 64 * 16 : 64 * 36 * 4); }
template <int BPW, bool SW, int NWT, bool LANE = false, bool LOOP = false, int PRO = PRO_COPY, int CTW = 1, bool CP = false>
static void launch_q4k_kr_t(tts_hip_backend * be, const GemvJob & job, unsigned gx, unsigned gy = 1) {
    static const int tail_bits[5] = {0, KR_TAIL_RES | KR_TAIL_FOLD, KR_TAIL_RES | KR_TAIL_FOLD | KR_TAIL_BESIDE, KR_TAIL_RES, KR_TAIL_FOLD};
    GemvJob j = job;
    j.kr_tail = tail_bits[be->gemv_kr_tail];
    if constexpr (PRO == PRO_COPY && CTW == 1 && !CP) {
        if (j.pro == PRO_LN) return launch_q4k_kr_t<BPW, SW, NWT, LANE, LOOP, PRO_LN>(be, j, gx, gy);
        if (j.pro == PRO_QUANT) return launch_q4k_kr_t<BPW, SW, NWT, LANE, LOOP, PRO_QUANT>(be, j, gx, gy);
    }
    if constexpr (SW && !LOOP && BPW <= 3 && CTW == 1) {
        if (be->gemv_kr_loop && gx > (unsigned)be->cus && gy == 1) {
            launch_q4k_kr_t<BPW, SW, NWT, LANE, true, PRO>(be, j, (unsigned)be->cus, gy);
            return;
        }
    }
    static std::atomic<uint32_t> attr_done{0};
    set_lds_attr_once(attr_done, be->device, (const void *)k_gemv_q4K_kr<BPW, SW, NWT, LANE, LOOP, PRO, CTW, CP>);
    size_t lds = q4k_kr_lds((CP ? 2 : CTW) * (j.bq_tile ? j.bq_tile : j.bq_bytes), SW || CP);
    if constexpr (!SW && !LOOP && CTW == 1 && !CP && BPW == 1 && NWT == 4) {
        if ((j.kr_tail & KR_TAIL_FOLD) && j.K == 4 * QK_K) {
            const size_t ops = lds - 64 * 36 * 4;
            lds = (j.kr_tail & KR_TAIL_BESIDE) ? ops + KR_FOLD_BYTES : std::max(ops, (size_t)KR_FOLD_BYTES);
        }
    }
    const dim3 blk(64 * NWT * ((SW || CP) ? 2 : 1));
    if (be->profile_gemv) {
        hipEvent_t e0, e1;
        profile_pair(be, e0, e1);
        hipExtLaunchKernelGGL((k_gemv_q4K_kr<BPW, SW, NWT, LANE, LOOP, PRO, CTW, CP>), dim3(gx, gy), blk, (uint32_t)lds, be->stream, e0, e1, 0u, j);
        profile_push(be, e0, e1, gemv_bytes(j), TTS_TYPE_Q4_K);
        return;
    }
    hipLaunchKernelGGL((k_gemv_q4K_kr<BPW, SW, NWT, LANE, LOOP, PRO, CTW, CP>), dim3(gx, gy), blk, lds, be->stream, j);
}

static size_t q4k_pf_lds(int64_t nb) { return (size_t)((((16 * nb + 1) * (2 * PF_SLOT + 32 + 4)) + 1023) & ~(int64_t)1023); }
template <int NB, bool LANE, int NW>
static void launch_q4k_pf_nw(tts_hip_backend * be, const GemvJob & j, unsigned gy) {
    static std::atomic<uint32_t> attr_done{0};
    set_lds_attr_once(attr_done, be->device, (const void *)k_gemm_q4K_pf<NB, LANE, NW>);
    const unsigned gx = (unsigned)((job_rows(j) / 16 + NW * PF_RS - 1) / (NW * PF_RS));
    hipLaunchKernelGGL((k_gemm_q4K_pf<NB, LANE, NW>), dim3(gx, gy), dim3(64 * NW), (uint32_t)q4k_pf_lds(NB), be->stream, j);
}
template <int NB, bool LANE>
static void launch_q4k_pf_t(tts_hip_backend * be, const GemvJob & j, unsigned gy) {
    if (be->gemm_pf_nw == 8) launch_q4k_pf_nw<NB, LANE, 8>(be, j, gy);
    else launch_q4k_pf_nw<NB, LANE, 4>(be, j, gy);
}

static bool launch_gemm_q4k_kr(tts_hip_backend * be, const GemvJob & job, size_t lo_res = SIZE_MAX) {
    if (!be->gemv_kr || !be->gemv_mf_prequant || job.wtype != TTS_TYPE_Q4_K || job.M <= 8 || job.epi == EPI_SWIGLU || job.dbg) return false;
    if (job.pro != PRO_QUANT && job.pro != PRO_LN) return false;
    if (job.pro == PRO_LN && job.K > 4 * 1024) return false;
    const int64_t nb = job.K / QK_K;
    if (nb != 4 && nb != 8 && nb != 12 && nb != 16) return false;
    for (int m = 0; m <= job.nmat; ++m)
        if (job_roff(job, m) % 16) return false;
    const int64_t ink_m = be->gemm_kr_ink & 0xFFFF;
    const bool ink = ink_m > 0 && job.M <= ink_m && job.K <= 4 * 1024 && !job.dbg &&
                     (job.pro == PRO_LN || job.xcs == job.K) && (!(be->gemm_kr_ink & 0x10000) || job.pro == PRO_QUANT);
    const bool pf = be->gemm_pf > 0 && job.M >= be->gemm_pf && !ink;
    const int64_t tile = pf ? (int64_t)q4k_pf_lds(nb) : (((16 * nb + 1) * (2 * QK_K + 32 + 4)) + 1023) & ~(int64_t)1023;
    const int64_t nct = (job.M + 15) / 16;
    if (q4k_kr_lds(tile, false) > 160 * 1024) return false;
    const char * xs0 = (const char *)job.x;
    const char * xs1 = xs0 + 4 * (size_t)((job.M - 1) * job.xcs + job.K);
    const size_t lo = lo_res != SIZE_MAX ? lo_res
                      : (xs0 >= be->scratch && xs0 < be->scratch + be->scratch_size) ? (size_t)(xs1 - be->scratch) : 0;
    const int64_t avail = lo < be->scratch_size ? (int64_t)(be->scratch_size - lo) : 0;
    if (tile * nct > avail || (lo == 0 && (size_t)(tile * nct + 4 * job.K * job.M) > be->scratch_size) || nct > 65535) {
        const int64_t per = (lo ? avail / tile : (int64_t)be->scratch_size / (tile + 16 * 4 * job.K)) * 16;
        if (per < 16 || job.rep_mat >= 0) return false;
        for (int64_t m0 = 0; m0 < job.M; m0 += per) {
            GemvJob j = job;
            j.M = job.M - m0 < per ? job.M - m0 : per;
            if (job.lnout) j.lnout = job.lnout + m0 * job.locs;
            j.x = job.x + m0 * job.xcs;
            for (int i = 0; i < job.nmat; ++i) j.Y[i] = job.Y[i] + m0 * job.ycs[i];
        if (job.yoff) j.yoff = job.yoff + m0;
            if (job.res) j.res = job.res + m0 * job.rcs;
            if (!launch_gemm_q4k_kr(be, j, lo)) return false;
        }
        return true;
    }
    GemvJob j = job;
    j.bq_tile = tile;
    j.bq_bytes = tile * nct;
    j.bq_slot = pf ? PF_SLOT : 0;
    if (ink) {
        j.bq = nullptr;
    } else {
        j.bq = be->scratch + be->scratch_size - j.bq_bytes;
        const dim3 qg((unsigned)((nb + 3) / 4), (unsigned)j.M);
        if (j.pro == PRO_LN) hipLaunchKernelGGL(k_quant_mf<PRO_LN>, qg, dim3(64), 0, be->stream, j);
        else hipLaunchKernelGGL(k_quant_mf<PRO_QUANT>, qg, dim3(64), 0, be->stream, j);
        TTS_HIP_CHECK(hipGetLastError());
        j.pro = PRO_COPY;
        j.lnout = nullptr;
    }
    const unsigned gx = (unsigned)(job_rows(j) / 16), gy = (unsigned)nct;
    j.xcd_cols = be->gemm_kr_xcd && nct > 1 ? 1 : 0;
    const bool ct2 = be->gemm_kr_ct2 && !ink && nct >= 2 && (nb == 4 || nb == 8) && q4k_kr_lds(2 * tile, false) <= 160 * 1024;
    const bool cp = be->gemm_kr_cp && !ink && nct >= 2 && (nb == 4 || nb == 8) && q4k_kr_lds(2 * tile, true) <= 160 * 1024;
    auto go = [&](auto LANE) {
        constexpr bool L = decltype(LANE)::value;
        if (pf) {
            switch (nb) {
                case 4: launch_q4k_pf_t<4, L>(be, j, gy); break;
                case 8: launch_q4k_pf_t<8, L>(be, j, gy); break;
                case 12: launch_q4k_pf_t<12, L>(be, j, gy); break;
                default: launch_q4k_pf_t<16, L>(be, j, gy); break;
            }
            return;
        }
        if (cp) {
            const unsigned gy2 = (unsigned)((nct + 1) / 2);
            if (nb == 4) launch_q4k_kr_t<1, false, 4, L, false, PRO_COPY, 1, true>(be, j, gx, gy2);
            else launch_q4k_kr_t<2, false, 4, L, false, PRO_COPY, 1, true>(be, j, gx, gy2);
            return;
        }
        if (ct2) {
            const unsigned gy2 = (unsigned)((nct + 1) / 2);
            if (nb == 4) launch_q4k_kr_t<1, false, 4, L, false, PRO_COPY, 2>(be, j, gx, gy2);
            else launch_q4k_kr_t<2, false, 4, L, false, PRO_COPY, 2>(be, j, gx, gy2);
            return;
        }
        const int walk = be->gemm_kr_walk;
        if (walk > 0 && nct > 4 && gx > (unsigned)walk && !ink) {
            switch (nb) {
                case 4: launch_q4k_kr_t<1, false, 4, L, true>(be, j, (unsigned)walk, gy); break;
                case 8: launch_q4k_kr_t<2, false, 4, L, true>(be, j, (unsigned)walk, gy); break;
                case 12: launch_q4k_kr_t<3, false, 4, L, true>(be, j, (unsigned)walk, gy); break;
                default: launch_q4k_kr_t<4, false, 4, L, true>(be, j, (unsigned)walk, gy); break;
            }
            return;
        }
        const bool nw8 = be->gemm_kr_nw == 8;
        switch (nb) {
            case 4: launch_q4k_kr_t<1, false, 4, L>(be, j, gx, gy); break;
            case 8: nw8 ? launch_q4k_kr_t<1, false, 8, L>(be, j, gx, gy) : launch_q4k_kr_t<2, false, 4, L>(be, j, gx, gy); break;
            case 12: launch_q4k_kr_t<3, false, 4, L>(be, j, gx, gy); break;
            default: nw8 ? launch_q4k_kr_t<2, false, 8, L>(be, j, gx, gy) : launch_q4k_kr_t<4, false, 4, L>(be, j, gx, gy); break;
        }
    };
    if (j.tiled) go(std::false_type{});
    else go(std::true_type{});
    TTS_HIP_CHECK(hipGetLastError());
    return true;
}
static bool launch_q4k_kr(tts_hip_backend * be, const GemvJob & j) {
    if (!be->gemv_kr || j.M > 8) return false;
    if (j.pro != PRO_COPY && !((j.pro == PRO_QUANT || j.pro == PRO_LN) && j.K <= 4 * 1024 && !j.bq_tile)) return false;
    const bool sw = j.epi == EPI_SWIGLU;
    if (!sw) {
        for (int m = 0; m <= j.nmat; ++m)
            if (job_roff(j, m) % 16) return false;
    } else if (j.N % 16) {
        return false;
    }
    if (q4k_kr_lds(j.bq_bytes, sw) > 160 * 1024) return false;
    const int64_t T = sw ? j.N / 16 : job_rows(j) / 16;
    if (T < 1 || T > 0x7fffffff) return false;
    const unsigned gx = (unsigned)T;
    switch (j.K / QK_K) {
        case 4: sw ? launch_q4k_kr_t<1, true, 4>(be, j, gx) : launch_q4k_kr_t<1, false, 4>(be, j, gx); return true;
        case 8: sw ? launch_q4k_kr_t<2, true, 4>(be, j, gx) : launch_q4k_kr_t<2, false, 4>(be, j, gx); return true;
        case 12: sw ? launch_q4k_kr_t<3, true, 4>(be, j, gx) : launch_q4k_kr_t<3, false, 4>(be, j, gx); return true;
        case 16: sw ? launch_q4k_kr_t<4, true, 4>(be, j, gx) : launch_q4k_kr_t<4, false, 4>(be, j, gx); return true;
        case 32: if (sw) return false; launch_q4k_kr_t<4, false, 8>(be, j, gx); return true;
        default: return false;
    }
}

static size_t q4k_ks_lds(int64_t M, int64_t nb) {
// ... 1075 lines not shown
            while (RW > 1 && q80_lds(MC, j.K, RW) > 64 * 1024) RW /= 2;
            const size_t lds = q80_lds(MC, j.K, RW) + (j.pro ? QK_K + 64 : 0);
            const unsigned grid = (unsigned)((j.N + RW - 1) / RW);
            if (j.pro == PRO_LN) hipLaunchKernelGGL((k_gemv_q8_0<MC, PRO_LN>), dim3(grid, nmat), dim3(256), lds, be->stream, j, RW);
            else if (j.pro == PRO_QUANT) hipLaunchKernelGGL((k_gemv_q8_0<MC, PRO_QUANT>), dim3(grid, nmat), dim3(256), lds, be->stream, j, RW);
            else hipLaunchKernelGGL(k_gemv_q8_0<MC>, dim3(grid, nmat), dim3(256), lds, be->stream, j, RW);
        } break;
        case TTS_TYPE_F16: {
            const unsigned grid = (unsigned)((j.N + 3) / 4);
            hipLaunchKernelGGL((k_gemv_float<MC, true>), dim3(grid, nmat), dim3(256), 0, be->stream, j);
        } break;
        default: {
            const unsigned grid = (unsigned)((j.N + 3) / 4);
            hipLaunchKernelGGL((k_gemv_float<MC, false>), dim3(grid, nmat), dim3(256), 0, be->stream, j);
        } break;
    }
}

__global__ void k_spin(long long ticks) {
    const long long t0 = (long long)__builtin_amdgcn_s_memrealtime();
    while ((long long)__builtin_amdgcn_s_memrealtime() - t0 < ticks) __builtin_amdgcn_s_sleep(2);
}

void launch_profile_spin(tts_hip_backend * be, double us) {
    hipLaunchKernelGGL(k_spin, dim3(1), dim3(64), 0, be->stream, (long long)(us * 100.0));
    TTS_HIP_CHECK(hipGetLastError());
}

void launch_gemv_job(tts_hip_backend * be, const GemvJob & job) {
    const bool prof = be->profile_gemv && job.wtype != TTS_TYPE_Q4_K && !(job.wtype == TTS_TYPE_Q8_0 && job.M <= 8 && q80s_ok(be, job)) &&
                      !(job.wtype == TTS_TYPE_Q5_0 && job.M <= 8 && q50s_ok(be, job)) &&
                      !(job.wtype == TTS_TYPE_Q4_0 && job.M <= 8 && q40s_ok(be, job));
    hipEvent_t e0 = nullptr, e1 = nullptr;
    if (prof) {
        profile_pair(be, e0, e1);
        TTS_HIP_CHECK(hipEventRecord(e0, be->stream));
    }
    const int64_t K = job.K;
    if (job.wtype == TTS_TYPE_F32 && job.M > 8 && gemm_f32_ok(job)) {
        launch_gemm_f32(be, job);
        if (prof) {
            TTS_HIP_CHECK(hipEventRecord(e1, be->stream));
            profile_push(be, e0, e1, gemv_bytes(job), job.wtype);
        }
        return;
    }
    if (job.wtype == TTS_TYPE_Q8_0 && job.M > 8 && job.aq.vtype == TTS_TYPE_Q8_0 && !job.hetero && be->gemm_q8) {
        launch_gemm_q8_0(be, job);
        TTS_HIP_CHECK(hipGetLastError());
        if (prof) {
            TTS_HIP_CHECK(hipEventRecord(e1, be->stream));
            profile_push(be, e0, e1, gemv_bytes(job), job.wtype);
        }
        return;
    }
    if (job.wtype == TTS_TYPE_Q5_0 && job.M > 8 && job.aq.vtype == TTS_TYPE_Q8_0 && !job.hetero && be->gemm_q5) {
        launch_gemm_q5_0(be, job);
        TTS_HIP_CHECK(hipGetLastError());
        if (prof) {
            TTS_HIP_CHECK(hipEventRecord(e1, be->stream));
            profile_push(be, e0, e1, gemv_bytes(job), job.wtype);
        }
        return;
    }
    if (job.wtype == TTS_TYPE_Q4_0 && job.M > 8 && job.aq.vtype == TTS_TYPE_Q8_0 && !job.hetero && be->gemm_q4_0) {
        launch_gemm_q4_0(be, job);
        TTS_HIP_CHECK(hipGetLastError());
        if (prof) {
            TTS_HIP_CHECK(hipEventRecord(e1, be->stream));
            profile_push(be, e0, e1, gemv_bytes(job), job.wtype);
        }
        return;
    }
    if (job.wtype == TTS_TYPE_Q6_K) {
        launch_gemv_q6k(be, job);
        TTS_HIP_CHECK(hipGetLastError());
        if (prof) {
            TTS_HIP_CHECK(hipEventRecord(e1, be->stream));
            profile_push(be, e0, e1, gemv_bytes(job), job.wtype);
        }
        return;
    }
    if (job.M > 8 && launch_gemm_q4k_kr(be, job)) return;
    if (q4k_ks_eligible(be, job)) {
        launch_q4k_ks(be, job);
        TTS_HIP_CHECK(hipGetLastError());
        return;
    }
    if (q4k_mf_eligible(be, job)) {
        launch_q4k_mf(be, job);
        TTS_HIP_CHECK(hipGetLastError());
        return;
    }
    if (job.epi == EPI_SWIGLU) {
        fprintf(stderr, "tts_hip: SwiGLU GEMV epilogue needs the matrix-core Q4_K kernel\n");
        abort();
    }
    const int64_t cmax = job.wtype == TTS_TYPE_Q4_K ? q4k_max_cols(K) : 8;
    for (int64_t m0 = 0; m0 < job.M; m0 += cmax) {
        const int64_t mc = job.M - m0 < cmax ? job.M - m0 : cmax;
        GemvJob j = job;
        j.M = mc;
        if (job.lnout) j.lnout = job.lnout + m0 * job.locs;
        if (job.aq.vtype == TTS_TYPE_Q8_K) {
            j.aq.qs = job.aq.qs + m0 * K;
            j.aq.d = job.aq.d + m0 * (K / QK_K);
            j.aq.bsums = job.aq.bsums + m0 * (K / 32);
        } else if (job.aq.vtype == TTS_TYPE_Q8_0) {
            j.aq.qs = job.aq.qs + m0 * K;
            j.aq.d = job.aq.d + m0 * (K / QK8_0);
        } else if (job.aq.vtype == TTS_TYPE_F16) {
            j.aq.qs = job.aq.qs + m0 * K * 2;
        }
        if (job.x) j.x = job.x + m0 * job.xcs;
        for (int i = 0; i < job.nmat; ++i) j.Y[i] = job.Y[i] + m0 * job.ycs[i];
        if (job.yoff) j.yoff = job.yoff + m0;
        if (job.res) j.res = job.res + m0 * job.rcs;
        switch (mc) {
            case 1: launch_gemv_mc<1>(be, j); break;
            case 2: launch_gemv_mc<2>(be, j); break;
            case 3: case 4: launch_gemv_mc<4>(be, j); break;
            default: launch_gemv_mc<8>(be, j); break;
        }
    }
    TTS_HIP_CHECK(hipGetLastError());
    if (prof) {
        TTS_HIP_CHECK(hipEventRecord(e1, be->stream));
        profile_push(be, e0, e1, gemv_bytes(job), job.wtype);
    }
}

}
```

### tts.cpp_amd/ttship/__init__.py

```python
import ctypes
import os
import pathlib

_HERE = pathlib.Path(__file__).resolve().parent
PKG_ROOT = _HERE.parent
REPO_ROOT = PKG_ROOT.parent
LIB_PATH = PKG_ROOT / "lib" / "libtts_hip.so"

F32, F16, Q4_0, Q5_0, Q8_0, Q4_K, Q6_K, Q8_K, I32 = 0, 1, 2, 6, 8, 12, 14, 15, 26
QUANT_MIX_Q4_K_M = 1
PROF_ATTN = 39

OPS = ["NONE", "DUP", "ADD", "SUB", "MUL", "DIV", "SQR", "SQRT", "SIN", "COS", "SUM_ROWS", "REPEAT",
       "CONCAT", "NORM", "RMS_NORM", "MUL_MAT", "SCALE", "CPY", "CONT", "RESHAPE", "VIEW", "PERMUTE",
       "TRANSPOSE", "GET_ROWS", "SOFT_MAX", "ROPE", "CLAMP", "CONV_TRANSPOSE_1D", "IM2COL", "UPSCALE",
       "PAD", "LEAKY_RELU", "UNARY", "CUMSUM", "MOD", "ROUND", "STFT", "ISTFT", "MAP_CUSTOM3", "MAP_CUSTOM2"]
OP = {n: i for i, n in enumerate(OPS)}
FUSE = {"LN": 1, "GROUP": 2, "KV": 4, "EPI": 8, "HEADS": 16, "ATTN": 32, "LSTM": 64, "SNAKE": 128, "EMBED": 256, "CONV": 512, "ADAIN": 1024, "XATTN": 2048, "MCPY": 4096, "CONTREAD": 8192}
FUSE_ALL = sum(FUSE.values())
UNARY = {"ABS": 0, "NEG": 1, "TANH": 2, "RELU": 3, "SIGMOID": 4, "GELU": 5, "SILU": 6, "EXP": 7}

OPT = {"FUSION": 0, "PROFILE_GEMV": 1, "GRAPHS": 2, "CONV_F32ACC": 3, "CONVT_LDS": 4, "ATTN_SPLIT": 5, "KV_PREFETCH": 6, "KV_PREFETCH_BLOCKS": 7, "Q4K_TILE_BYTES": 8, "GEMV_DEBUG": 10, "GEMV_UNIQUE": 11, "CONV_SPLIT": 12, "GEMV_KS": 13, "ATTN_FUSED": 14, "ATTN_PV16": 15, "Q4K_DUAL_BYTES": 16, "GEMV_RSPLIT": 17, "GEMM_Q8": 18, "BGEMM_F32": 19, "CU_PARTITION": 20, "GEMV_PREQUANT": 21, "GEMV_KRELAY": 22, "ATTN_KS": 23, "ATTN_PV8": 24, "GEMV_NW_MIN": 25, "GEMV_KRELAY_LOOP": 26, "GEMV_Q80_PRO": 27, "GEMV_Q80_SLAB": 28, "GEMV_Q80_RW": 29, "GEMM_Q8_STAGED": 30, "GEMV_KR_INKERNEL": 31, "GEMV_F32_WIDE": 32, "ATTN_PV_MP": 33, "GEMM_KR_NW": 34, "GEMM_KR_INKERNEL": 35, "GEMM_KR_CT2": 36, "COALESCE": 37, "GEMM_KR_XCD": 38, "GEMM_KR_CP": 39, "GEMM_KR_WALK": 40, "GEMM_PF": 41, "GEMM_PF_NW": 42, "ATTN_ONE": 43, "GEMV_KR_TAIL": 44, "GEMV_Q50_SLAB": 45, "GEMV_Q50_RW": 46, "GEMM_Q5": 47, "GEMM_Q5_STAGED": 48, "GEMV_Q40_SLAB": 49, "GEMV_Q40_RW": 50, "GEMM_Q4_0": 51, "GEMM_Q4_0_STAGED": 52, "CONV_VFMA": 53, "CONV_TILE96": 54, "CONV_PACK": 55, "CONVT_PACK": 56, "CONV_XREG": 57}
ATTN_SPLIT_DEFAULT = 128
ATTN_ONE_DEFAULT = 1
GEMV_KR_TAIL_DEFAULT = 1
ATTN_FUSED_ON = 128

TYPE_SIZE = {F32: 4, F16: 2, Q4_K: 144, Q6_K: 210, Q8_0: 34, Q5_0: 22, Q4_0: 18, I32: 4}
BLCK_SIZE = {F32: 1, F16: 1, Q4_K: 256, Q6_K: 256, Q8_0: 32, Q5_0: 32, Q4_0: 32, I32: 1}


class TtsTensor(ctypes.Structure):
    pass


TtsTensor._fields_ = [
    ("type", ctypes.c_int32),
    ("op", ctypes.c_int32),
    ("ne", ctypes.c_int64 * 4),
    ("nb", ctypes.c_uint64 * 4),
    ("op_params", ctypes.c_int32 * 16),
    ("src", ctypes.POINTER(TtsTensor) * 4),
    ("view_src", ctypes.POINTER(TtsTensor)),
    ("view_offs", ctypes.c_uint64),
    ("data", ctypes.c_void_p),
    ("flags", ctypes.c_int32),
    ("pad_", ctypes.c_int32),
    ("name", ctypes.c_char * 64),
]


class BackendIface(ctypes.Structure):
    _fields_ = [
        ("ctx", ctypes.c_void_p),
        ("name", ctypes.c_char_p),
        ("alloc", ctypes.c_void_p),
        ("free", ctypes.c_void_p),
        ("set", ctypes.c_void_p),
        ("set_tensor", ctypes.c_void_p),
        ("get", ctypes.c_void_p),
        ("memset", ctypes.c_void_p),
        ("compute", ctypes.c_void_p),
        ("synchronize", ctypes.c_void_p),
        ("prepare", ctypes.c_void_p),
        ("launch", ctypes.c_void_p),
        ("set_async", ctypes.c_void_p),
        ("copy", ctypes.c_void_p),
        ("greedy_step", ctypes.c_void_p),
        ("sample_step", ctypes.c_void_p),
    ]


class Sampling(ctypes.Structure):
    _fields_ = [
        ("temperature", ctypes.c_float),
        ("top_p", ctypes.c_float),
        ("repetition_penalty", ctypes.c_float),
        ("top_k", ctypes.c_int32),
        ("do_sample", ctypes.c_int32),
        ("pad_", ctypes.c_int32),
        ("seed", ctypes.c_uint64),
    ]


def sampling(**kw):
    c = Sampling()
    lib().tts_sampling_default(ctypes.byref(c))
    for k, v in kw.items():
        setattr(c, k, v)
    return c


def call_seed(seed, stream, call):
    return int(lib().tts_sampler_call_seed(seed, stream, call))


def host_sample(cfg, logits, call_seed_, last=None, count=None):
    import numpy as np
    lg = np.ascontiguousarray(logits, dtype=np.float32)
    NH, V = lg.shape
    out = np.zeros(NH, dtype=np.int32)
    if last is None:
        last = np.full(NH, -1, dtype=np.int32)
    if count is None:
        count = np.zeros(NH, dtype=np.int32)
# ... 450 lines not shown
            raise RuntimeError("tts_hip_backend_iface failed")
        if reference_flow:
            for f in ("prepare", "launch", "set_async", "copy", "greedy_step", "sample_step"):
                setattr(it, f, None)
        return it

    def alloc(self, nbytes):
        p = self.L.tts_hip_buffer_alloc(self.ptr, nbytes)
        if not p:
            raise MemoryError(f"tts_hip_buffer_alloc({nbytes}) failed")
        return p

    def free(self, p):
        self.L.tts_hip_buffer_free(self.ptr, p)

    def set(self, dev, host_arr):
        st = self.L.tts_hip_tensor_set(self.ptr, dev, host_arr.ctypes.data, host_arr.nbytes)
        if st != 0:
            raise RuntimeError(f"tensor_set failed {st}")

    def get(self, host_arr, dev):
        st = self.L.tts_hip_tensor_get(self.ptr, host_arr.ctypes.data, dev, host_arr.nbytes)
        if st != 0:
            raise RuntimeError(f"tensor_get failed {st}")

    def sample_step(self, logits, cfg, call, rep_state=None, step=100, bos=-2, eos=-3, eos_seen=None):
        import numpy as np
        lg = np.ascontiguousarray(logits, dtype=np.float32)
        B, NH, V = lg.shape
        rs = np.ascontiguousarray(rep_state if rep_state is not None else np.tile(np.array([-1, 0], np.int32), B * NH), dtype=np.int32)
        es = np.ascontiguousarray(eos_seen if eos_seen is not None else np.zeros(B * NH, np.int32), dtype=np.int32)
        bufs = [self.alloc(n) for n in (lg.nbytes, rs.nbytes, es.nbytes, B * NH * 4, B * NH * 4)]
        try:
            self.set(bufs[0], lg)
            self.set(bufs[1], rs)
            self.set(bufs[2], es)
            st = self.L.tts_hip_sample_step(self.ptr, bufs[0], B, NH, V, ctypes.byref(cfg), call, bufs[1], step, bos, eos, bufs[2], bufs[3], bufs[4])
            if st != 0:
                raise RuntimeError(f"tts_hip_sample_step failed {st}")
            hist = np.zeros((B, NH), np.int32)
            nxt = np.zeros((NH, B), np.int32)
            self.get(hist, bufs[3])
            self.get(nxt, bufs[4])
            self.get(rs, bufs[1])
            self.get(es, bufs[2])
            return hist, nxt, es, rs
        finally:
            for b in bufs:
                self.free(b)

    def quantize(self, wtype, x):
        import numpy as np
        x = np.ascontiguousarray(x, dtype=np.float32)
        N, K = x.shape
        rs = K // BLCK_SIZE[wtype] * TYPE_SIZE[wtype]
        dx, dq = self.alloc(x.nbytes), self.alloc(N * rs)
        try:
            self.set(dx, x)
            st = self.L.tts_hip_quantize(self.ptr, wtype, dx, dq, N, K)
            if st != 0:
                raise RuntimeError(f"tts_hip_quantize failed {st}")
            out = np.empty(N * rs, dtype=np.uint8)
            self.get(out, dq)
            return out
        finally:
            self.free(dx)
            self.free(dq)

    def sync(self):
        if self.L.tts_hip_synchronize(self.ptr) != 0:
            raise RuntimeError("synchronize failed")

    def set_option(self, opt, value):
        self.L.tts_hip_set_option(self.ptr, opt, value)

    def gemv_stats(self, wtype=-1, reset=True):
        ms = ctypes.c_double()
        n = ctypes.c_int64()
        b = ctypes.c_double()
        self.L.tts_hip_gemv_stats(self.ptr, wtype, ctypes.byref(ms), ctypes.byref(n), ctypes.byref(b), 1 if reset else 0)
        return ms.value, n.value, b.value

    def counters(self):
        out = (ctypes.c_int64 * 10)()
        n = self.L.tts_hip_counters(self.ptr, out, 10)
        keys = ("graph_updates", "graph_instantiations", "lstm_chains", "lstm_steps", "plan_wait_ns",
                "cap_plan_ns", "cap_launch_ns", "cap_update_ns", "conv_pack_images", "conv_pack_bytes")
        return {keys[i]: int(out[i]) for i in range(n)}

    def close(self):
        if self.ptr:
            self.L.tts_hip_backend_free(self.ptr)
            self.ptr = None


def runner_weights(n_fn, w_fn, ptr):
    import numpy as np
    out = {}
    for i in range(n_fn(ptr)):
        name = ctypes.create_string_buffer(128)
        ne = (ctypes.c_int64 * 4)()
        ty = ctypes.c_int32()
        n = w_fn(ptr, i, name, 128, ne, ctypes.byref(ty), None, 0)
        if ty.value not in (F32, F16):
            continue
        a = np.empty(n, dtype=np.uint8)
        w_fn(ptr, i, name, 128, ne, ctypes.byref(ty), a.ctypes.data, n)
        a = a.view(np.float32 if ty.value == F32 else np.float16).astype(np.float32)
        shape = [int(v) for v in reversed(list(ne))]
        while len(shape) > 1 and shape[0] == 1:
            shape.pop(0)
        out[name.value.decode()] = a.reshape(shape)
    return out


class _Runner:
    PREFIX = None
    TYPED_WEIGHTS = True

    def _fn(self, name):
        return getattr(self.L, f"{self.PREFIX}_{name}")

    def weight_bytes(self):
        return self._fn("weight_bytes")(self.ptr)

    def weights(self):
        n_fn, w_fn = self._fn("n_weights"), self._fn("weight")
        if self.TYPED_WEIGHTS:
            return runner_weights(n_fn, w_fn, self.ptr)
        return runner_weights(n_fn, lambda ptr, i, name, cap, ne, ty, dst, n: w_fn(ptr, i, name, cap, ne, dst, n), self.ptr)

    def weights_raw(self):
        import numpy as np
        w_fn = self._fn("weight" if self.TYPED_WEIGHTS else "weight_raw")
        out = {}
        for i in range(self._fn("n_weights")(self.ptr)):
            name = ctypes.create_string_buffer(128)
            ne = (ctypes.c_int64 * 4)()
            ty = ctypes.c_int32()
            n = w_fn(self.ptr, i, name, 128, ne, ctypes.byref(ty), None, 0)
            a = np.empty(n, dtype=np.uint8)
            if w_fn(self.ptr, i, name, 128, ne, ctypes.byref(ty), a.ctypes.data, n) != n:
                raise RuntimeError(f"reading weight {name.value.decode()} failed")
            out[name.value.decode()] = (ty.value, tuple(ne), a)
        return out

    def set_weight(self, i, data):
        import numpy as np
        d = np.ascontiguousarray(data).view(np.uint8).reshape(-1)
        if self._fn("set_weight")(self.ptr, i, d.ctypes.data, d.nbytes) != 0:
            raise RuntimeError(f"setting weight {i} failed ({d.nbytes} bytes)")

    def plan_stats(self, mask=None):
        n = ctypes.c_int32()
        p = self._fn("graph")(self.ptr, ctypes.byref(n))
        return plan_stats(p, n.value, FUSE_ALL if mask is None else mask)

    def node(self, i, cap=1 << 26):
        import numpy as np
        op, ty = ctypes.c_int32(), ctypes.c_int32()
        ne = (ctypes.c_int64 * 4)()
        buf = np.empty(cap // 4, dtype=np.float32)
        n = self._fn("node")(self.ptr, i, ctypes.byref(op), ctypes.byref(ty), ne, buf.ctypes.data, cap)
        data = buf[: n // 4].copy() if n else None
        return OPS[op.value], ty.value, tuple(ne), data

    def named(self, name, dtype="float32", lead=()):
        import numpy as np
        get = self._fn("get_node")
        n = get(self.ptr, *lead, name.encode(), None, 0)
# ... 845 lines not shown
```

Before: 125.2.

## Quantize fused cross-attention output directly into the K-relay GEMM operand tiles

Adds a new fused Q-projection plus cross-attention kernel that handles four heads per 1024-thread block. It writes the attention output straight into the Q8_K operand tiles the following Q4_K K-relay GEMM reads, kept in the shadow buffer. A planner pass links each qualifying attention item to its single-consumer output projection, and that projection then skips its own quantize prologue and the column copy. This removes the f32 output write, the separate quantization kernel launch and its re-read of the activations. In exchange it adds a larger, more complex kernel with narrow eligibility (head dim 64, heads a multiple of four, M in the K-relay range) and an abort path if the GEMM cannot accept pre-quantized tiles.

Result: no change. 126.7 (median of 3 runs) (+1.2%).

```diff
diff --git a/include/tts_hip.h b/include/tts_hip.h
--- a/include/tts_hip.h
+++ b/include/tts_hip.h
@@ -228,6 +228,7 @@
     TTS_HIP_OPT_CONV_PACK = 55,
     TTS_HIP_OPT_CONVT_PACK = 56,
     TTS_HIP_OPT_CONV_XREG = 57,
+    TTS_HIP_OPT_ATTN_OPERANDS = 58,
     TTS_HIP_OPT_COALESCE = 37,
 };
 enum tts_fuse_bits {
@@ -272,6 +273,7 @@
                         int32_t * next);
 int tts_sampling_device_ok(const tts_sampling * cfg, int32_t V);
 int tts_hip_counters(tts_hip_backend_t backend, int64_t * out, int n);
+int64_t tts_hip_attn_operands_read(tts_hip_backend_t backend, const float * x, int64_t K, int64_t M, void * dst, size_t bytes);
 
 int tts_hip_gemv(tts_hip_backend_t backend, int type, const void * w, const float * x, float * y,
                  int64_t K, int64_t N, int64_t M);
diff --git a/tts.cpp_amd/csrc/backend.hip b/tts.cpp_amd/csrc/backend.hip
--- a/tts.cpp_amd/csrc/backend.hip
+++ b/tts.cpp_amd/csrc/backend.hip
@@ -185,6 +185,8 @@
         if (e[0] >= '0' && e[0] <= '1' && !e[1]) be->convt_pack = e[0] - '0';
     if (const char * e = getenv("TTS_HIP_OPT_CONV_XREG"))
         if (e[0] >= '0' && e[0] <= '1' && !e[1]) be->conv_xreg = e[0] - '0';
+    if (const char * e = getenv("TTS_HIP_OPT_ATTN_OPERANDS"))
+        if (e[0] >= '0' && e[0] <= '3' && !e[1]) be->attn_operands = e[0] - '0';
     be->conv_part_doubles = (size_t)8 << 20;
     TTS_HIP_CHECK(hipMalloc((void **)&be->conv_part, be->conv_part_doubles * sizeof(double)));
     be->lstm_floats = kLstmFloats;
@@ -969,17 +971,41 @@
         case TTS_HIP_OPT_GEMM_KR_WALK: be->gemm_kr_walk = value < 0 ? 0 : value; return 0;
         case TTS_HIP_OPT_GEMM_PF: be->gemm_pf = value < 0 ? 0 : value; return 0;
         case TTS_HIP_OPT_GEMM_PF_NW: be->gemm_pf_nw = value == 8 ? 8 : 4; return 0;
+        case TTS_HIP_OPT_ATTN_OPERANDS:
+            if (value < 0 || value > 3) return TTS_STATUS_BAD_ARG;
+            be->attn_operands = value;
+            return 0;
         case TTS_HIP_OPT_KV_PREFETCH_BLOCKS: be->kv_prefetch_blocks = value > 0 ? value : 1; return 0;
         default: return TTS_STATUS_BAD_ARG;
     }
 }
 
+extern "C" int64_t tts_hip_attn_operands_read(tts_hip_backend_t be, const float * x, int64_t K, int64_t M, void * dst, size_t bytes) {
+    if (!be || K <= 0 || M <= 0 || K % 256) return TTS_STATUS_BAD_ARG;
+    const int64_t tile = gemm_q4k_kr_operand_tile(be, K, M);
+    const size_t need = (size_t)(tile * ((M + 15) / 16));
+    if (tile <= 0 || need > be->shadow_size || need > be->scratch_size) return TTS_STATUS_UNSUPPORTED;
+    if (!dst) return (int64_t)need;
+    if (bytes != need) return TTS_STATUS_BAD_ARG;
+    hipSetDevice(be->device);
+    const char * src = (const char *)be->shadow;
+    if (x) {
+        char * bq = be->scratch + be->scratch_size - need;
+        launch_quant_mf_tiles(be, x, K, M, bq, tile);
+        src = bq;
+    }
+    TTS_HIP_CHECK(hipStreamSynchronize(be->stream));
+    TTS_HIP_CHECK(hipMemcpy(dst, src, need, hipMemcpyDeviceToHost));
+    return (int64_t)need;
+}
+
 extern "C" int tts_hip_counters(tts_hip_backend_t be, int64_t * out, int n) {
     if (!be || !out) return TTS_STATUS_BAD_ARG;
-    const int64_t v[10] = {be->graph_updates, be->graph_instantiations, be->lstm_chains, be->lstm_steps, be->plan_wait_ns,
-                           be->cap_plan_ns, be->cap_launch_ns, be->cap_update_ns, (int64_t)g_packs_n.load(), (int64_t)g_packs_bytes.load()};
+    const int64_t v[11] = {be->graph_updates, be->graph_instantiations, be->lstm_chains, be->lstm_steps, be->plan_wait_ns,
+                           be->cap_plan_ns, be->cap_launch_ns, be->cap_update_ns, (int64_t)g_packs_n.load(), (int64_t)g_packs_bytes.load(),
+                           be->attn_opnd_folds};
     int k = 0;
-    for (; k < n && k < 10; ++k) out[k] = v[k];
+    for (; k < n && k < 11; ++k) out[k] = v[k];
     return k;
 }
 
diff --git a/tts.cpp_amd/csrc/graph_exec.hip b/tts.cpp_amd/csrc/graph_exec.hip
--- a/tts.cpp_amd/csrc/graph_exec.hip
+++ b/tts.cpp_amd/csrc/graph_exec.hip
@@ -134,6 +134,7 @@
     bool shadow = false;
     int xattn = -1;
     bool fused = false;
+    int opnd_to = -1;
     const tts_tensor *q = nullptr, *k = nullptr, *v = nullptr, *mask = nullptr, *out = nullptr;
     const tts_tensor * bias = nullptr;
     bool stage = false;
@@ -352,6 +353,7 @@
         if (mask & TTS_FUSE_LN) fuse_ln_into_gemv();
         link_attn_shadow();
         if (mask & TTS_FUSE_XATTN) fuse_xattn();
+        link_attn_operands();
         tmark("post");
         if (timing) fprintf(stderr, "plan %d nodes ms:%s\n", n, tbuf);
     }
@@ -369,6 +371,31 @@
             const tts_tensor * x = G.mms[0]->src[1];
             if (x->data != A.out->data || !contiguous(x) || tbytes(x) != tbytes(A.out)) continue;
             A.shadow = G.x_shadow = true;
+        }
+    }
+
+    void link_attn_operands() {
+        for (int i = 0; i < n; ++i) {
+            const int a = act[i];
+            if (a <= 0 || items[a - 1].kind != Item::ATTN) continue;
+            Item & A = items[a - 1];
+            if (!A.shadow || A.bias) continue;
+            if (A.q->ne[0] != 64 || A.q->ne[1] != 1 || A.q->ne[2] % 4) continue;
+            const int nx = next_real(i);
+            Item & G = items[act[nx] - 1];
+            if (G.mms.size() != 1 || G.epi == EPI_SWIGLU || G.xattn >= 0 || G.xsrc) continue;
+            const tts_tensor * mm = G.mms[0];
+            const tts_tensor * W = mm->src[0];
+            const int64_t H = A.q->ne[2], B = A.q->ne[3];
+            if (W->ne[0] != 64 * H || nel(mm->src[1]) != 64 * H * B || W->ne[1] % 16) continue;
+            const tts_tensor * t = mm->src[1];
+            bool one = sole_consumer(t) == mm;
+            for (int hops = 0; one && t != A.out && hops < 4; ++hops) {
+                one = is_view(t->op) && t->src[0] && sole_consumer(t->src[0]) == t;
+                t = t->src[0];
+            }
+            if (!one || t != A.out) continue;
+            A.opnd_to = act[nx] - 1;
         }
     }
 
@@ -2015,8 +2042,10 @@
 }
 
 static int run_gemv_item(tts_hip_backend * be, const Item & it, const Item * xattn = nullptr, const ItemTab * tab = nullptr,
-                         const ItemTab * xtab = nullptr) {
+                         const ItemTab * xtab = nullptr, const Item * opnd = nullptr) {
     const tts_tensor * mm0 = it.mms[0];
+    const bool pre = be->opnd_for == &it;
+    be->opnd_for = nullptr;
     const tts_tensor * a0 = mm0->src[0];
     tts_tensor bx;
     if (it.xsrc) {
@@ -2088,7 +2117,7 @@
             j.M = NB;
         }
         x_hit |= ((uintptr_t)j.x & 15) != 0 || (j.xcs & 3) != 0;
-        if (x_hit) {
+        if (x_hit && !pre) {
             if (!ensure_scratch(be, (size_t)(4 * j.K * j.M))) return TTS_STATUS_ALLOC_FAILED;
             launch_copy_cols(be, (float *)be->scratch, j.x, j.K, j.xcs, j.M);
             be->aq.src = nullptr;
@@ -2142,6 +2171,20 @@
             xa.P = (int)A.k->ne[1];
             xa.H = (int)A.q->ne[2];
             xa.B = (int)A.q->ne[3];
+            if (opnd && (be->attn_operands & 1) && !bc && xa.H % 4 == 0) {
+                const tts_tensor * Wo = opnd->mms[0]->src[0];
+                const int64_t tile = Wo->type == TTS_TYPE_Q4_K && (Wo->flags & TTS_FLAG_REPACKED)
+                                         ? gemm_q4k_kr_operand_tile(be, Wo->ne[0], xa.B) : 0;
+                if (tile > 0 && (size_t)(tile * ((xa.B + 15) / 16)) <= be->shadow_size) {
+                    xa.oq = (char *)be->shadow;
+                    xa.oq_tile = tile;
+                    xa.out2 = nullptr;
+                    xa.out = nullptr;
+                    be->opnd_for = opnd;
+                    be->opnd_tile = tile;
+                    be->attn_opnd_folds++;
+                }
+            }
             if (bc) {
                 if (xtab && xtab->koff) xa.k.ne[3] = NB, xa.k.nb[3] = 0;
                 else batch_td(*bc, xa.k);
@@ -2208,6 +2251,11 @@
             if (tmp) break;
         }
         if (jj.hetero) jj.N = 0;
+        if (pre) {
+            jj.pro = PRO_COPY;
+            jj.bq = (const char *)be->shadow;
+            jj.bq_tile = be->opnd_tile;
+        }
         if (jj.wtype == TTS_TYPE_Q6_K && !gemv_q6k_ok(jj)) return TTS_STATUS_UNSUPPORTED;
         launch_gemv_job(be, jj);
     }
@@ -2323,7 +2371,8 @@
     switch (it.kind) {
         case Item::GEMV:
             return run_gemv_item(be, it, it.xattn >= 0 ? &items[it.xattn] : nullptr, tab,
-                                 be->bat && it.xattn >= 0 ? &be->bat->tabs[it.xattn] : nullptr);
+                                 be->bat && it.xattn >= 0 ? &be->bat->tabs[it.xattn] : nullptr,
+                                 it.xattn >= 0 && items[it.xattn].opnd_to >= 0 ? &items[items[it.xattn].opnd_to] : nullptr);
         case Item::ATTN:
             if (it.fused) return 0;
             return run_attn_item(be, it, tab);
diff --git a/tts.cpp_amd/csrc/hip_internal.h b/tts.cpp_amd/csrc/hip_internal.h
--- a/tts.cpp_amd/csrc/hip_internal.h
+++ b/tts.cpp_amd/csrc/hip_internal.h
@@ -284,7 +284,11 @@
     const int64_t * voff = nullptr;
     const int64_t * moff = nullptr;
     const int * pseq = nullptr;
-};
+    char * oq = nullptr;
+    int64_t oq_tile = 0;
+};
+int64_t gemm_q4k_kr_operand_tile(const tts_hip_backend * be, int64_t K, int64_t M);
+void launch_quant_mf_tiles(tts_hip_backend * be, const float * x, int64_t K, int64_t M, char * bq, int64_t tile);
 
 constexpr int EMBED_MAX_TERMS = 16;
 struct BatchCls {
@@ -395,6 +399,10 @@
     int64_t gemv_kr_ink = 0;
     int gemm_kr_walk = 0;
     int gemm_pf = 64;
+    int attn_operands = 1;
+    const void * opnd_for = nullptr;
+    int64_t opnd_tile = 0;
+    int64_t attn_opnd_folds = 0;
     int gemm_pf_nw = 4;
     int gemm_kr_cp = 0;
     int gemm_kr_xcd = 0;
diff --git a/tts.cpp_amd/csrc/k_gemv.hip b/tts.cpp_amd/csrc/k_gemv.hip
--- a/tts.cpp_amd/csrc/k_gemv.hip
+++ b/tts.cpp_amd/csrc/k_gemv.hip
@@ -1694,7 +1694,154 @@
     if (a.out2) a.out2[(int64_t)b * a.H * HD + orow] = (float)o;
 }
 
+template <int PRO>
+__global__ __launch_bounds__(1024) void k_gemv_q4K_xattn4(GemvJob j, XAttnArgs a) {
+    constexpr int HD = 64, NW = 16, F = HD / 4, VB = 8;
+    __shared__ __attribute__((aligned(16))) int8_t xq_s[5 * QK_K];
+    __shared__ float xd_s[8];
+    __shared__ __attribute__((aligned(16))) int16_t xs_s[5 * 8];
+    __shared__ float s_q[4 * HD];
+    __shared__ __attribute__((aligned(16))) float s_o[4 * HD];
+    const int g = blockIdx.x, b = blockIdx.y;
+    const int lane = threadIdx.x & 63, wave = __builtin_amdgcn_readfirstlane(threadIdx.x >> 6);
+    const int l = lane & 7, s = lane >> 3;
+    const int nb = (int)(j.K / QK_K);
+    const int h = 4 * g + (wave & 3);
+    const int P = a.pseq ? a.pseq[b] : a.P;
+    const int p = min(lane, P - 1);
+    const int bk = b / (a.B / (int)a.k.ne[3]), bv = b / (a.B / (int)a.v.ne[3]);
+    const char * kbase = a.k.data + (int64_t)h * a.k.nb[2] + (int64_t)bk * a.k.nb[3] + (a.koff ? a.koff[b] : 0);
+    const char * vbase = a.v.data + (int64_t)h * a.v.nb[2] + (int64_t)bv * a.v.nb[3] + (a.voff ? a.voff[b] : 0);
+    u32x4 hdr[2][4], q[2][4];
+    {
+        const int64_t row = (int64_t)g * (4 * HD) + wave * 16 + s;
+        const uint8_t * wr = j.W[0] + row * j.w_row_bytes;
+        auto load_pass = [&](auto PS) __attribute__((always_inline)) {
+            constexpr int ps = decltype(PS)::value;
+#pragma unroll
+            for (int u = 0; u < 4; ++u) {
+                const int64_t bo = (int64_t)ps * 8 * j.w_row_bytes + (int64_t)min(u, nb - 1) * 144;
+                hdr[ps][u] = TTS_WLOAD((const u32x4 *)(wr + bo));
+                q[ps][u] = TTS_WLOAD((const u32x4 *)(wr + bo + 16 + l * 16));
+            }
+        };
+        using P0 = std::integral_constant<int, 0>;
+        using P1 = std::integral_constant<int, 1>;
+        ProOv ov;
+        ov.nwaves = NW;
+        ov.xcol = j.x + (int64_t)b * j.xcs;
+        ov.lncol = j.lnout && g == 0 ? j.lnout + (int64_t)b * j.locs : nullptr;
+        if constexpr (PRO == PRO_LN) {
+            if (wave == 0) {
+                q4k_prologue<PRO, 4>(j, nb, xq_s, xd_s, xs_s, nullptr, nullptr, [&]() { load_pass(P0{}); }, ov);
+                load_pass(P1{});
+            } else {
+                load_pass(P0{});
+                load_pass(P1{});
+            }
+        } else {
+            auto mid = [&]() {
+                load_pass(P0{});
+                load_pass(P1{});
+            };
+            q4k_prologue<PRO, 4>(j, nb, xq_s, xd_s, xs_s, nullptr, nullptr, mid, ov);
+        }
+    }
+    __syncthreads();
+    {
+        float sums = 0.f, sumf = 0.f;
+#pragma unroll
+        for (int u = 0; u < 4; ++u) q4k_block(hdr[0][u], q[0][u], xq_s, xs_s, xd_s, min(u, nb - 1), l, u < nb, sums, sumf);
+        const float tot = q4k_octet_total(sumf, sums);
+        if (l == 0) s_q[wave * 16 + s] = tot;
+    }
+    float4 kr[F];
+    float vv[VB];
+    float mk = 0.f;
+    if (wave < 4) {
+#pragma unroll
+        for (int c = 0; c < F; ++c) kr[c] = *(const float4 *)(kbase + (int64_t)p * a.k.nb[1] + 16 * c);
+#pragma unroll
+        for (int u = 0; u < VB; ++u) vv[u] = *(const float *)(vbase + (int64_t)lane * a.v.nb[1] + (int64_t)min(u, P - 1) * a.v.nb[0]);
+        mk = *(a.mask ? a.mask + (a.moff ? a.moff[b] : (int64_t)b * a.mbs) + p : (const float *)kbase);
+    }
+    {
+        float sums = 0.f, sumf = 0.f;
+#pragma unroll
+        for (int u = 0; u < 4; ++u) q4k_block(hdr[1][u], q[1][u], xq_s, xs_s, xd_s, min(u, nb - 1), l, u < nb, sums, sumf);
+        const float tot = q4k_octet_total(sumf, sums);
+        if (l == 0) s_q[wave * 16 + 8 + s] = tot;
+    }
+    __syncthreads();
+    if (wave < 4) {
+        const float * sq = s_q + wave * HD;
+        double acc = 0.0;
+#pragma unroll
+        for (int c = 0; c < F; ++c) {
+            acc += (double)__fmul_rn(kr[c].x, sq[4 * c + 0]);
+            acc += (double)__fmul_rn(kr[c].y, sq[4 * c + 1]);
+            acc += (double)__fmul_rn(kr[c].z, sq[4 * c + 2]);
+            acc += (double)__fmul_rn(kr[c].w, sq[4 * c + 3]);
+        }
+        float w = __fmul_rn((float)acc, a.scale);
+        if (a.mask) w = __fadd_rn(w, __fmul_rn(1.0f, mk));
+        if (lane >= P) w = -INFINITY;
+        float mx = w;
+        mx = fmaxf(mx, dpp_f32<DPP_XOR1>(mx));
+        mx = fmaxf(mx, dpp_f32<DPP_XOR2>(mx));
+        mx = fmaxf(mx, dpp_f32<DPP_HALF_MIRROR>(mx));
+        mx = fmaxf(mx, dpp_f32<DPP_MIRROR>(mx));
+        mx = fmaxf(fmaxf(__int_as_float(__builtin_amdgcn_readlane(__float_as_int(mx), 0)), __int_as_float(__builtin_amdgcn_readlane(__float_as_int(mx), 16))),
+                   fmaxf(__int_as_float(__builtin_amdgcn_readlane(__float_as_int(mx), 32)), __int_as_float(__builtin_amdgcn_readlane(__float_as_int(mx), 48))));
+        const float e = lane < P ? cr_expf(__fsub_rn(w, mx)) : 0.f;
+        double sum = 0.0;
+        for (int i = 0; i < P; ++i) sum += (double)__int_as_float(__builtin_amdgcn_readlane(__float_as_int(e), i));
+        const float pr = __fmul_rn(e, (float)(1.0 / sum));
+        double o = 0.0;
+        for (int i0 = 0; i0 < P; i0 += VB) {
+            if (i0 > 0) {
+#pragma unroll
+                for (int u = 0; u < VB; ++u) vv[u] = *(const float *)(vbase + (int64_t)lane * a.v.nb[1] + (int64_t)min(i0 + u, P - 1) * a.v.nb[0]);
+                TTS_PIN_LOADS();
+            }
+#pragma unroll
+            for (int u = 0; u < VB; ++u) {
+                if (i0 + u >= P) break;
+                const float pi = __int_as_float(__builtin_amdgcn_readlane(__float_as_int(pr), i0 + u));
+                o += (double)__fmul_rn(pi, vv[u]);
+            }
+        }
+        const int64_t orow = (int64_t)h * HD + lane;
+        if (a.out) a.out[(int64_t)b * (a.obs ? a.obs : (int64_t)a.H * HD) + orow] = (float)o;
+        if (a.out2) a.out2[(int64_t)b * a.H * HD + orow] = (float)o;
+        s_o[wave * HD + lane] = (float)o;
+    }
+    __syncthreads();
+    if (threadIdx.x < 16) {
+        const int nbo = a.H / 4, ct = b >> 4;
+        const int Mt = min(16, a.B - 16 * ct), nslot = Mt * nbo + 1;
+        _Float16 * b16 = (_Float16 *)(a.oq + (size_t)ct * a.oq_tile);
+        _Float16 * sb = b16 + (size_t)nslot * QK_K;
+        float * xd = (float *)(sb + (size_t)nslot * 16);
+        const int slot = (b & 15) * nbo + g;
+        float v[16];
+#pragma unroll
+        for (int k = 0; k < 4; ++k) {
+            const float4 t4 = *(const float4 *)(s_o + 16 * lane + 4 * k);
+            v[4 * k] = t4.x, v[4 * k + 1] = t4.y, v[4 * k + 2] = t4.z, v[4 * k + 3] = t4.w;
+        }
+        q8k_row_block_mf(v, lane, b16 + (size_t)slot * QK_K, sb + (size_t)slot * 16, xd + slot);
+    }
+}
+
 void launch_gemv_q4K_xattn(tts_hip_backend * be, const GemvJob & j, const XAttnArgs & a) {
+    if (a.oq) {
+        const dim3 grid4((unsigned)(a.H / 4), (unsigned)a.B);
+        if (j.pro == PRO_LN) hipLaunchKernelGGL(k_gemv_q4K_xattn4<PRO_LN>, grid4, dim3(1024), 0, be->stream, j, a);
+        else hipLaunchKernelGGL(k_gemv_q4K_xattn4<PRO_QUANT>, grid4, dim3(1024), 0, be->stream, j, a);
+        TTS_HIP_CHECK(hipGetLastError());
+        return;
+    }
     const dim3 grid((unsigned)a.H, (unsigned)a.B);
     if (j.pro == PRO_LN) hipLaunchKernelGGL(k_gemv_q4K_xattn<PRO_LN>, grid, dim3(576), 0, be->stream, j, a);
     else hipLaunchKernelGGL(k_gemv_q4K_xattn<PRO_QUANT>, grid, dim3(576), 0, be->stream, j, a);
@@ -2667,21 +2814,53 @@
     else launch_q4k_pf_nw<NB, LANE, 4>(be, j, gy);
 }
 
+static bool launch_gemm_q4k_kr_tiles(tts_hip_backend * be, const GemvJob & job, int64_t tile, int64_t nct, bool ink, bool pf);
+static int64_t q4k_kr_tile_bytes(int64_t nb) { return (((16 * nb + 1) * (2 * QK_K + 32 + 4)) + 1023) & ~(int64_t)1023; }
+int64_t gemm_q4k_kr_operand_tile(const tts_hip_backend * be, int64_t K, int64_t M) {
+    if (!be->gemv_kr || !be->gemv_mf_prequant || M <= 8 || K % QK_K) return 0;
+    const int64_t nb = K / QK_K;
+    if (nb != 4 && nb != 8 && nb != 12 && nb != 16) return 0;
+    if ((be->gemm_kr_ink & 0xFFFF) > 0 && M <= (be->gemm_kr_ink & 0xFFFF)) return 0;
+    if (be->gemm_pf > 0 && M >= be->gemm_pf) return 0;
+    const int64_t tile = q4k_kr_tile_bytes(nb);
+    if (q4k_kr_lds(tile, false) > 160 * 1024 || (M + 15) / 16 > 65535) return 0;
+    return tile;
+}
+void launch_quant_mf_tiles(tts_hip_backend * be, const float * x, int64_t K, int64_t M, char * bq, int64_t tile) {
+    GemvJob j;
+    j.wtype = TTS_TYPE_Q4_K;
+    j.K = K;
+    j.M = M;
+    j.x = x;
+    j.xcs = K;
+    j.pro = PRO_QUANT;
+    j.bq = bq;
+    j.bq_tile = tile;
+    j.bq_bytes = tile * ((M + 15) / 16);
+    const dim3 qg((unsigned)((K / QK_K + 3) / 4), (unsigned)M);
+    hipLaunchKernelGGL(k_quant_mf<PRO_QUANT>, qg, dim3(64), 0, be->stream, j);
+    TTS_HIP_CHECK(hipGetLastError());
+}
 static bool launch_gemm_q4k_kr(tts_hip_backend * be, const GemvJob & job, size_t lo_res = SIZE_MAX) {
     if (!be->gemv_kr || !be->gemv_mf_prequant || job.wtype != TTS_TYPE_Q4_K || job.M <= 8 || job.epi == EPI_SWIGLU || job.dbg) return false;
-    if (job.pro != PRO_QUANT && job.pro != PRO_LN) return false;
+    const bool pre = job.pro == PRO_COPY && job.bq && job.bq_tile > 0;
+    if (job.pro != PRO_QUANT && job.pro != PRO_LN && !pre) return false;
     if (job.pro == PRO_LN && job.K > 4 * 1024) return false;
     const int64_t nb = job.K / QK_K;
     if (nb != 4 && nb != 8 && nb != 12 && nb != 16) return false;
     for (int m = 0; m <= job.nmat; ++m)
         if (job_roff(job, m) % 16) return false;
     const int64_t ink_m = be->gemm_kr_ink & 0xFFFF;
-    const bool ink = ink_m > 0 && job.M <= ink_m && job.K <= 4 * 1024 && !job.dbg &&
+    const bool ink = !pre && ink_m > 0 && job.M <= ink_m && job.K <= 4 * 1024 && !job.dbg &&
                      (job.pro == PRO_LN || job.xcs == job.K) && (!(be->gemm_kr_ink & 0x10000) || job.pro == PRO_QUANT);
     const bool pf = be->gemm_pf > 0 && job.M >= be->gemm_pf && !ink;
-    const int64_t tile = pf ? (int64_t)q4k_pf_lds(nb) : (((16 * nb + 1) * (2 * QK_K + 32 + 4)) + 1023) & ~(int64_t)1023;
+    const int64_t tile = pf ? (int64_t)q4k_pf_lds(nb) : q4k_kr_tile_bytes(nb);
     const int64_t nct = (job.M + 15) / 16;
     if (q4k_kr_lds(tile, false) > 160 * 1024) return false;
+    if (pre) {
+        if (pf || tile != job.bq_tile || nct > 65535) return false;
+        return launch_gemm_q4k_kr_tiles(be, job, tile, nct, false, false);
+    }
     const char * xs0 = (const char *)job.x;
     const char * xs1 = xs0 + 4 * (size_t)((job.M - 1) * job.xcs + job.K);
     const size_t lo = lo_res != SIZE_MAX ? lo_res
@@ -2702,13 +2881,17 @@
         }
         return true;
     }
+    return launch_gemm_q4k_kr_tiles(be, job, tile, nct, ink, pf);
+}
+static bool launch_gemm_q4k_kr_tiles(tts_hip_backend * be, const GemvJob & job, int64_t tile, int64_t nct, bool ink, bool pf) {
+    const int64_t nb = job.K / QK_K;
     GemvJob j = job;
     j.bq_tile = tile;
     j.bq_bytes = tile * nct;
     j.bq_slot = pf ? PF_SLOT : 0;
     if (ink) {
         j.bq = nullptr;
-    } else {
+    } else if (job.pro != PRO_COPY) {
         j.bq = be->scratch + be->scratch_size - j.bq_bytes;
         const dim3 qg((unsigned)((nb + 3) / 4), (unsigned)j.M);
         if (j.pro == PRO_LN) hipLaunchKernelGGL(k_quant_mf<PRO_LN>, qg, dim3(64), 0, be->stream, j);
@@ -3950,6 +4133,10 @@
         return;
     }
     if (job.M > 8 && launch_gemm_q4k_kr(be, job)) return;
+    if (job.pro == PRO_COPY && job.bq_tile > 0) {
+        fprintf(stderr, "tts_hip: pre-quantized Q4_K product (K %lld, M %lld) has no K-relay GEMM\n", (long long)job.K, (long long)job.M);
+        abort();
+    }
     if (q4k_ks_eligible(be, job)) {
         launch_q4k_ks(be, job);
         TTS_HIP_CHECK(hipGetLastError());
diff --git a/tts.cpp_amd/ttship/__init__.py b/tts.cpp_amd/ttship/__init__.py
--- a/tts.cpp_amd/ttship/__init__.py
+++ b/tts.cpp_amd/ttship/__init__.py
@@ -20,7 +20,7 @@
 FUSE_ALL = sum(FUSE.values())
 UNARY = {"ABS": 0, "NEG": 1, "TANH": 2, "RELU": 3, "SIGMOID": 4, "GELU": 5, "SILU": 6, "EXP": 7}
 
-OPT = {"FUSION": 0, "PROFILE_GEMV": 1, "GRAPHS": 2, "CONV_F32ACC": 3, "CONVT_LDS": 4, "ATTN_SPLIT": 5, "KV_PREFETCH": 6, "KV_PREFETCH_BLOCKS": 7, "Q4K_TILE_BYTES": 8, "GEMV_DEBUG": 10, "GEMV_UNIQUE": 11, "CONV_SPLIT": 12, "GEMV_KS": 13, "ATTN_FUSED": 14, "ATTN_PV16": 15, "Q4K_DUAL_BYTES": 16, "GEMV_RSPLIT": 17, "GEMM_Q8": 18, "BGEMM_F32": 19, "CU_PARTITION": 20, "GEMV_PREQUANT": 21, "GEMV_KRELAY": 22, "ATTN_KS": 23, "ATTN_PV8": 24, "GEMV_NW_MIN": 25, "GEMV_KRELAY_LOOP": 26, "GEMV_Q80_PRO": 27, "GEMV_Q80_SLAB": 28, "GEMV_Q80_RW": 29, "GEMM_Q8_STAGED": 30, "GEMV_KR_INKERNEL": 31, "GEMV_F32_WIDE": 32, "ATTN_PV_MP": 33, "GEMM_KR_NW": 34, "GEMM_KR_INKERNEL": 35, "GEMM_KR_CT2": 36, "COALESCE": 37, "GEMM_KR_XCD": 38, "GEMM_KR_CP": 39, "GEMM_KR_WALK": 40, "GEMM_PF": 41, "GEMM_PF_NW": 42, "ATTN_ONE": 43, "GEMV_KR_TAIL": 44, "GEMV_Q50_SLAB": 45, "GEMV_Q50_RW": 46, "GEMM_Q5": 47, "GEMM_Q5_STAGED": 48, "GEMV_Q40_SLAB": 49, "GEMV_Q40_RW": 50, "GEMM_Q4_0": 51, "GEMM_Q4_0_STAGED": 52, "CONV_VFMA": 53, "CONV_TILE96": 54, "CONV_PACK": 55, "CONVT_PACK": 56, "CONV_XREG": 57}
+OPT = {"FUSION": 0, "PROFILE_GEMV": 1, "GRAPHS": 2, "CONV_F32ACC": 3, "CONVT_LDS": 4, "ATTN_SPLIT": 5, "KV_PREFETCH": 6, "KV_PREFETCH_BLOCKS": 7, "Q4K_TILE_BYTES": 8, "GEMV_DEBUG": 10, "GEMV_UNIQUE": 11, "CONV_SPLIT": 12, "GEMV_KS": 13, "ATTN_FUSED": 14, "ATTN_PV16": 15, "Q4K_DUAL_BYTES": 16, "GEMV_RSPLIT": 17, "GEMM_Q8": 18, "BGEMM_F32": 19, "CU_PARTITION": 20, "GEMV_PREQUANT": 21, "GEMV_KRELAY": 22, "ATTN_KS": 23, "ATTN_PV8": 24, "GEMV_NW_MIN": 25, "GEMV_KRELAY_LOOP": 26, "GEMV_Q80_PRO": 27, "GEMV_Q80_SLAB": 28, "GEMV_Q80_RW": 29, "GEMM_Q8_STAGED": 30, "GEMV_KR_INKERNEL": 31, "GEMV_F32_WIDE": 32, "ATTN_PV_MP": 33, "GEMM_KR_NW": 34, "GEMM_KR_INKERNEL": 35, "GEMM_KR_CT2": 36, "COALESCE": 37, "GEMM_KR_XCD": 38, "GEMM_KR_CP": 39, "GEMM_KR_WALK": 40, "GEMM_PF": 41, "GEMM_PF_NW": 42, "ATTN_ONE": 43, "GEMV_KR_TAIL": 44, "GEMV_Q50_SLAB": 45, "GEMV_Q50_RW": 46, "GEMM_Q5": 47, "GEMM_Q5_STAGED": 48, "GEMV_Q40_SLAB": 49, "GEMV_Q40_RW": 50, "GEMM_Q4_0": 51, "GEMM_Q4_0_STAGED": 52, "CONV_VFMA": 53, "CONV_TILE96": 54, "CONV_PACK": 55, "CONVT_PACK": 56, "CONV_XREG": 57, "ATTN_OPERANDS": 58}
 ATTN_SPLIT_DEFAULT = 128
 ATTN_ONE_DEFAULT = 1
 GEMV_KR_TAIL_DEFAULT = 1
@@ -637,10 +637,10 @@
         return ms.value, n.value, b.value
 
     def counters(self):
-        out = (ctypes.c_int64 * 10)()
-        n = self.L.tts_hip_counters(self.ptr, out, 10)
+        out = (ctypes.c_int64 * 11)()
+        n = self.L.tts_hip_counters(self.ptr, out, 11)
         keys = ("graph_updates", "graph_instantiations", "lstm_chains", "lstm_steps", "plan_wait_ns",
-                "cap_plan_ns", "cap_launch_ns", "cap_update_ns", "conv_pack_images", "conv_pack_bytes")
+                "cap_plan_ns", "cap_launch_ns", "cap_update_ns", "conv_pack_images", "conv_pack_bytes", "attn_operand_folds")
         return {keys[i]: int(out[i]) for i in range(n)}
 
     def close(self):
```
